# ymingxie/PARQ

Hardware: AMD Instinct MI355X
Metric: decoder-iterations/sec (10 views, 256 queries, d=256) (higher is better)
Workload: dtype f32 (cross-attention scores: fp16 hi.hi + MX-fp8 e4m3 cross terms; P V: fp16 probabilities and values with a self-consistent normaliser; fp32 accumulation — 4e-6..1.5e-5 from float64 at the outputs on the reference's fixtures, the reference's own fp32 run: 6e-5..1.4e-4; guarded: rows on too few keys

## Files before the change

__graft_entry__.py:

```python
from __future__ import annotations

import glob
import os
import subprocess
import sys

ROOT = os.path.dirname(os.path.abspath(__file__))
CSRC = os.path.join(ROOT, "parq_amd", "csrc")
OUT = os.path.join(ROOT, "parq_amd", "_C", "libparq_hip.so")
OUT_DEV = os.path.join(ROOT, "parq_amd", "_C", "libparq_hip_dev.so")


def _hipcc():
    for c in (os.environ.get("HIPCC"), "/opt/rocm/bin/hipcc", "hipcc"):
        if c and (os.path.isabs(c) and os.path.exists(c) or not os.path.isabs(c)):
            return c
    return "hipcc"


def _compile(out: str, objdir: str, flags, force: bool) -> None:
    srcs = sorted(glob.glob(os.path.join(CSRC, "*.hip")))
    deps = srcs + glob.glob(os.path.join(CSRC, "*.hpp")) + [os.path.join(ROOT, "include", "parq_hip.h")]
    os.makedirs(objdir, exist_ok=True)
    if not force and os.path.exists(out) and all(os.path.getmtime(out) >= os.path.getmtime(d) for d in deps):
        print("[build] up to date:", out)
        return
    objs = []
    procs = []
    for s in srcs:
        o = os.path.join(objdir, os.path.basename(s)[:-4] + ".o")
        objs.append(o)
        cmd = [_hipcc(), "--offload-arch=gfx950", "-O3", "-std=c++17", "-fPIC"] + list(flags) + ["-c", s, "-o", o]
        print("[build]", " ".join(cmd))
        procs.append((cmd, subprocess.Popen(cmd)))
    for cmd, p in procs:
        if p.wait() != 0:
            raise RuntimeError("hipcc failed: %s" % " ".join(cmd))
    cmd = [_hipcc(), "--offload-arch=gfx950", "-shared", "-fPIC", "-o", out] + objs
    print("[build]", " ".join(cmd))
    subprocess.check_call(cmd)


def build_dev(force: bool = False) -> None:
    extra = os.environ.get("PARQ_DEV_EXTRA_FLAGS", "").split()
    _compile(OUT_DEV, os.path.join(os.path.dirname(OUT_DEV), "dev"), ["-DPARQ_DEV_PROBES"] + extra, force or bool(extra))


def build(force: bool = False) -> None:
    _compile(OUT, os.path.dirname(OUT), [], force)
    if ROOT not in sys.path:
        sys.path.insert(0, ROOT)
    import parq_amd
    from parq_amd import _lib
    lib = _lib.load()
    print("[build] loaded", lib.parq_version().decode(), "with", len(_lib.SYMBOLS), "entry points")


def smoke() -> None:
    if ROOT not in sys.path:
        sys.path.insert(0, ROOT)
    import numpy as np
    import torch
    from parq_amd import synth
    from parq_amd.decoder import PARQDecoder
    from oracle import parq_oracle as O

    assert torch.cuda.is_available(), "smoke() needs a GPU"
    cfg = synth.decoder_cfg(dim=256, queries=64, heads=4, ffn=768, layers=2)
    W = synth.make_decoder_weights(cfg, seed=5)
    sc = synth.make_scene(55, B=1, V=2, h=60, w=80, C=256)
    dec = PARQDecoder(cfg).eval()
    sd = dec.state_dict()
    for k in sd:
        src = k.replace("parq_module.decoder.mlp_heads.", "mlp_heads.")
        sd[k] = torch.from_numpy(W[src]).reshape(sd[k].shape)
    dec.load_state_dict(sd, strict=True)
    dec = dec.cuda()
    t = lambda a: torch.from_numpy(a).cuda()
    with torch.no_grad():
        outs = dec(t(sc["tokens"]), t(sc["camera"]), t(sc["T_camera_pseudoCam"]), t(sc["T_world_pseudoCam"]),
                   t(sc["T_world_local"]))
    torch.cuda.synchronize()
    od = O.OracleDecoder(cfg, W, synth.SCANNET_MEAN_SIZES)
    forced = [O.normalize(o["coord_pos"].cpu(), cfg.TRANSFORMER.SCALE) for o in outs]
    with torch.no_grad():
        ref = od.forward(sc["tokens"], sc["camera"], sc["T_camera_pseudoCam"], sc["T_world_pseudoCam"],
                         sc["T_world_local"], forced_refs=forced)
    worst = 0.0
    for k, (a, b) in enumerate(zip(outs, ref)):
        for key in b:
            bb = b[key].numpy().astype(np.float64)
            err = np.abs(a[key].cpu().numpy().astype(np.float64) - bb) / np.maximum(1.0, np.abs(bb))
            worst = max(worst, float(err.max()))
    print("[smoke] max err vs oracle (teacher-forced, 2 iterations): %.3e" % worst)
    assert worst < 1e-4, worst


if __name__ == "__main__":
    build()
    if len(sys.argv) > 1 and sys.argv[1] == "dev":
        build_dev()
    if len(sys.argv) > 1 and sys.argv[1] == "smoke":
        smoke()
```

include/parq_hip.h:

```cpp
#ifndef PARQ_HIP_H
#define PARQ_HIP_H

#include <stddef.h>
#include <stdint.h>

#ifdef __cplusplus
extern "C" {
#endif

typedef struct parq_ctx *parq_handle;
typedef void *parq_stream;

enum {
    PARQ_OK = 0,
    PARQ_ERR_ARG = 1,
    PARQ_ERR_HIP = 2,
    PARQ_ERR_STATE = 3,
    PARQ_ERR_WORKSPACE = 4
};

typedef struct parq_config {
    int32_t dim;
    int32_t num_queries;
    int32_t num_classes;
    int32_t num_heads;
    int32_t ffn_dim;
    int32_t num_layers;
    int32_t share_weights;
    int32_t num_mean_sizes;
    float scale[6];
} parq_config;

typedef struct parq_scene {
    int32_t B, V, h, w;
    const float *tokens;
    const float *camera;
    const float *T_camera_pseudoCam;
    const float *T_world_pseudoCam;
    const float *T_world_local;
} parq_scene;

typedef struct parq_outputs {
    float *pred_logits;
    float *center_unnormalized;
    float *size_unnormalized;
    float *ortho6d;
    float *sem_cls_prob;
    float *coord_pos;
} parq_outputs;

const char *parq_last_error(void);
const char *parq_version(void);

int parq_create(const parq_config *cfg, parq_handle *out);
int parq_destroy(parq_handle h);

int parq_set_weight(parq_handle h, const char *name, const float *dev, int64_t numel);
size_t parq_packed_weights_bytes(parq_handle h);
int parq_pack_weights(parq_handle h, void *arena, size_t arena_bytes, parq_stream stream);

int parq_set_attention_mode(parq_handle h, int32_t mode);

enum { PARQ_TOKENS_F32 = 0, PARQ_TOKENS_F16 = 1, PARQ_TOKENS_BF16 = 2 };
int parq_set_token_type(parq_handle h, int32_t type);
int parq_set_head_tiers(parq_handle h, uint32_t safe_mask, int32_t poison_on_peaked);
int parq_set_seam_fusion(parq_handle h, int32_t on);
int parq_set_range_mirror(parq_handle h, int32_t *host_visible_flag);
int32_t parq_mirror_take(int32_t *host_visible_flag);
int parq_set_progress(parq_handle h, int32_t *host_visible_word, int32_t epoch);

size_t parq_workspace_bytes(parq_handle h, int32_t B, int32_t V, int32_t hh, int32_t ww);

int parq_forward(parq_handle h, const parq_scene *scene, void *workspace, size_t workspace_bytes,
                 const parq_outputs *outs, parq_stream stream);

typedef struct parq_graph *parq_graph_t;
int parq_forward_capture(parq_handle h, int32_t B, int32_t V, int32_t hh, int32_t ww, void *workspace, size_t workspace_bytes,
                         parq_stream stream, parq_graph_t *out);
int parq_forward_replay(parq_handle h, parq_graph_t g, const parq_scene *scene, void *workspace, size_t workspace_bytes,
                        const parq_outputs *outs, parq_stream stream);
int64_t parq_graph_nodes(parq_graph_t g);
int parq_graph_destroy(parq_graph_t g);

int parq_prepare(parq_handle h, const parq_scene *scene, void *workspace, size_t workspace_bytes,
                 parq_stream stream);
int parq_iterate(parq_handle h, const parq_scene *scene, void *workspace, size_t workspace_bytes,
                 int32_t layer_num, const float *ref_in, const parq_outputs *outs, float *ref_out,
                 parq_stream stream);

size_t parq_shard_exchange_floats(parq_handle h, int32_t B, int32_t which);
int parq_iterate_sharded(parq_handle h, const parq_scene *scene, void *workspace, size_t workspace_bytes, int32_t layer_num,
                         int32_t phase, const float *ref_in, const parq_outputs *outs, float *ref_out, const float *xchg_in,
                         float *xchg_out, int32_t nranks, parq_stream stream);

int parq_workspace_lookup(parq_handle h, int32_t B, int32_t V, int32_t hh, int32_t ww, const char *name,
                          size_t *offset_floats, size_t *numel);

enum {
    PARQ_PROF_KV_PROJ = 0, PARQ_PROF_PROJECT_SAMPLE = 1, PARQ_PROF_CROSS_ATTN = 2,
    PARQ_PROF_SELF_ATTN = 3, PARQ_PROF_LINEAR = 4, PARQ_PROF_OTHER = 5, PARQ_PROF_MERGE = 6, PARQ_PROF_COUNT = 7
};
int parq_profile_enable(parq_handle h, int32_t on);
int parq_profile_read(parq_handle h, int32_t which, double *total_ms, int64_t *launches);

typedef struct parq_output_grads {
    const float *pred_logits, *center_unnormalized, *size_unnormalized, *ortho6d;
} parq_output_grads;
int parq_set_dropout(parq_handle h, float p, uint32_t seed);
int parq_set_backward_batched(parq_handle h, int32_t on);
int parq_k_dropout_mask(parq_handle h, int32_t iteration, int32_t site, int64_t rows, int64_t cols, float *out,
                        parq_stream stream);
size_t parq_train_workspace_bytes(parq_handle h, int32_t B, int32_t V, int32_t hh, int32_t ww);
size_t parq_grad_arena_bytes(parq_handle h);
int parq_forward_train(parq_handle h, const parq_scene *scene, void *workspace, size_t workspace_bytes,
                       const parq_outputs *outs, parq_stream stream);
int parq_wait_iteration(parq_handle h, int32_t k);
int parq_backward(parq_handle h, const parq_scene *scene, void *workspace, size_t workspace_bytes, const parq_outputs *outs,
                  const parq_output_grads *grads, float *grad_arena, float *d_tokens, parq_stream stream);
int parq_arena_lookup(parq_handle h, const char *name, int64_t *offset, int64_t *rows, int64_t *cols, int64_t *ld);
int parq_grad_bucket(parq_handle h, int32_t bucket, int64_t *offset, int64_t *count);
int parq_backward_wait_bucket(parq_handle h, int32_t bucket, parq_stream stream);
int parq_set_backward_streams(parq_handle h, int32_t n);
int parq_set_deterministic(parq_handle h, int32_t on);

enum { PARQ_RAYPE_NCHW_OUT = 1, PARQ_RAYPE_NO_HIDDEN = 2, PARQ_RAYPE_WEIGHTS_CACHED = 4, PARQ_RAYPE_OUT_F16 = 8, PARQ_RAYPE_OUT_BF16 = 16 };
size_t parq_ray_pe_workspace_bytes(int32_t B, int32_t V, int32_t hh, int32_t ww, int32_t C, int32_t num_samples);
size_t parq_ray_pe_workspace_bytes_flags(int32_t B, int32_t V, int32_t hh, int32_t ww, int32_t C, int32_t num_samples,
                                         int32_t flags);
int parq_ray_pe(const float *camera, const float *T_camera_pseudoCam, const float *T_world_pseudoCam,
                const float *T_world_local, const float *w1, const float *b1, const float *w2, const float *b2,
                const float *scale6_host, float min_depth, float max_depth, int32_t num_samples, int32_t B,
                int32_t V, int32_t hh, int32_t ww, int32_t C, const float *features_nchw, float *tokens_out,
                int32_t flags, void *workspace, size_t workspace_bytes, parq_stream stream);

typedef struct {
    const float *level[4];
    int32_t h[4], w[4];
    int32_t layer;
} parq_fpn_levels;
int parq_ray_pe_fpn(const float *camera, const float *T_camera_pseudoCam, const float *T_world_pseudoCam,
                    const float *T_world_local, const float *w1, const float *b1, const float *w2, const float *b2,
                    const float *scale6_host, float min_depth, float max_depth, int32_t num_samples, int32_t B,
                    int32_t V, int32_t hh, int32_t ww, int32_t C, const parq_fpn_levels *levels, float *tokens_out,
                    int32_t flags, void *workspace, size_t workspace_bytes, parq_stream stream);
int parq_fpn_backward(const float *d_tokens, int32_t B, int32_t V, int32_t C, const parq_fpn_levels *levels, float *const d_level[4],
                      parq_stream stream);

size_t parq_ray_pe_backward_workspace_bytes(int32_t B, int32_t V, int32_t hh, int32_t ww, int32_t C, int32_t num_samples);
int parq_ray_pe_backward(const float *camera, const float *T_camera_pseudoCam, const float *T_world_pseudoCam,
                         const float *T_world_local, const float *w2, const float *scale6_host, float min_depth,
                         float max_depth, int32_t num_samples, int32_t B, int32_t V, int32_t hh, int32_t ww, int32_t C,
                         const float *d_tokens, const void *fwd_workspace, void *bwd_workspace, size_t bwd_workspace_bytes,
                         float *dw1, float *db1, float *dw2, float *db2, float *d_features_nchw, parq_stream stream);
enum { PARQ_RAYPE_BWD_DETERMINISTIC = 1 };
size_t parq_ray_pe_backward_workspace_bytes_flags(int32_t B, int32_t V, int32_t hh, int32_t ww, int32_t C, int32_t num_samples,
                                                  int32_t flags);
int parq_ray_pe_backward_flags(const float *camera, const float *T_camera_pseudoCam, const float *T_world_pseudoCam,
                               const float *T_world_local, const float *w2, const float *scale6_host, float min_depth,
                               float max_depth, int32_t num_samples, int32_t B, int32_t V, int32_t hh, int32_t ww, int32_t C,
                               const float *d_tokens, const void *fwd_workspace, void *bwd_workspace, size_t bwd_workspace_bytes,
                               float *dw1, float *db1, float *dw2, float *db2, float *d_features_nchw, int32_t flags,
                               parq_stream stream);

int parq_parse_pred(const float *center, const float *size, const float *ortho6d, const float *sem_cls_prob, int32_t B,
                    int32_t Q, int32_t num_classes, const float *track_scale6_host, int32_t for_vis, int32_t enable_nms,
                    float *obbs_out, unsigned char *mask_out, parq_stream stream);

int parq_obb_iou(const double *boxes_a, int64_t n_a_total, const double *boxes_b, int64_t n_b_total, const int64_t *segments,
                 int32_t S, int64_t total_pairs, double *iou3d_out, double *iou2d_out, parq_stream stream);

int parq_set_loss(const float *pred_logits, const float *center_unnormalized, const float *size_unnormalized, const float *ortho6d,
                  int32_t I, int32_t B, int32_t Q, int32_t num_classes, const float *t_center, const float *t_size, const float *t_rot,
                  const int32_t *t_label, const int32_t *t_sym, int32_t nmax, const int32_t *pairs, const float *pair_coef, int32_t P,
                  const float *row_weight, const float *class_weight, const float *loss_weight4_host, float *terms, float *g_logits,
                  float *g_center, float *g_size, float *g_ortho6d, int32_t *class_scratch, parq_stream stream);
enum { PARQ_SETLOSS_DETERMINISTIC = 1 };
size_t parq_set_loss_scratch_bytes(int32_t I, int32_t B, int32_t Q, int32_t P, int32_t flags);
int parq_set_loss_flags(const float *pred_logits, const float *center_unnormalized, const float *size_unnormalized, const float *ortho6d,
                        int32_t I, int32_t B, int32_t Q, int32_t num_classes, const float *t_center, const float *t_size, const float *t_rot,
                        const int32_t *t_label, const int32_t *t_sym, int32_t nmax, const int32_t *pairs, const float *pair_coef, int32_t P,
                        const float *row_weight, const float *class_weight, const float *loss_weight4_host, float *terms, float *g_logits,
                        float *g_center, float *g_size, float *g_ortho6d, int32_t *class_scratch, int32_t flags, parq_stream stream);


int parq_k_project_sample(const float *tokens, const float *T_camera_local, const float *camera,
                          const float *ref, const float *scale6_host, int32_t B, int32_t V, int32_t hh,
                          int32_t ww, int32_t C, int32_t Q, float *tgt, float *coord_pos,
                          parq_stream stream);

int parq_k_camera_local(const float *T_cp, const float *T_wp, const float *T_wl, int32_t B, int32_t V,
                        float *T_cl, parq_stream stream);

int parq_k_linear(const float *X, const float *X2, const float *W, const float *bias, const float *R,
                  float *Y, int32_t M, int32_t N, int32_t K, int32_t relu, parq_stream stream);

int parq_k_linear_half(const float *X, const float *X2, const float *W, const float *bias, const float *R,
                       float *Y, int32_t M, int32_t N, int32_t K, int32_t relu, void *scratch, size_t scratch_bytes,
                       parq_stream stream);

size_t parq_k_attention_scratch_bytes(int32_t B, int32_t H, int32_t Lq, int32_t Lk, int32_t dh);
int parq_k_attention(const float *q, const float *k, const float *v, float *out, int32_t B, int32_t H,
                     int32_t Lq, int32_t Lk, int32_t dh, void *scratch, size_t scratch_bytes,
                     parq_stream stream);

size_t parq_k_attention_split_scratch_bytes(int32_t B, int32_t H, int32_t Lq, int32_t Lk);
int parq_k_attention_split(const float *q, const float *k, const float *v, float *out, int32_t B, int32_t H,
                           int32_t Lq, int32_t Lk, void *scratch, size_t scratch_bytes, parq_stream stream);

int parq_k_attention_split8(const float *q, const float *k, const float *v, float *out, int32_t B, int32_t H,
                            int32_t Lq, int32_t Lk, void *scratch, size_t scratch_bytes, parq_stream stream);

size_t parq_k_attention_split256_scratch_bytes(int32_t B, int32_t H, int32_t Lq, int32_t Lk);
int parq_k_attention_split256(const float *q, const float *k, const float *v, float *out, int32_t B, int32_t H,
                              int32_t Lq, int32_t Lk, void *scratch, size_t scratch_bytes, parq_stream stream);

size_t parq_k_attention_half_scratch_bytes(int32_t B, int32_t H, int32_t Lq, int32_t Lk);
int parq_k_attention_half(const float *q, const float *k, const float *v, float *out, int32_t B, int32_t H,
                          int32_t Lq, int32_t Lk, int32_t bf16, void *scratch, size_t scratch_bytes,
                          parq_stream stream);

int parq_k_layernorm(const float *X, const float *gamma, const float *beta, float *Y, int32_t M,
                     int32_t C, float eps, parq_stream stream);

#ifdef __cplusplus
}
#endif
#endif
```

parq_amd/_lib.py:

```python
from __future__ import annotations

import ctypes as C
import os

import torch

_HERE = os.path.dirname(os.path.abspath(__file__))
LIB_PATH = os.path.join(_HERE, "_C", "libparq_hip.so")
DEV_LIB_PATH = os.path.join(_HERE, "_C", "libparq_hip_dev.so")

PROF_KV_PROJ, PROF_PROJECT_SAMPLE, PROF_CROSS_ATTN, PROF_SELF_ATTN, PROF_LINEAR, PROF_OTHER, PROF_MERGE = range(7)
PROF_NAMES = ["kv_proj", "project_sample", "cross_attn", "self_attn", "linear", "other", "cross_attn_merge"]


class ParqConfig(C.Structure):
    _fields_ = [("dim", C.c_int32), ("num_queries", C.c_int32), ("num_classes", C.c_int32),
                ("num_heads", C.c_int32), ("ffn_dim", C.c_int32), ("num_layers", C.c_int32),
                ("share_weights", C.c_int32), ("num_mean_sizes", C.c_int32), ("scale", C.c_float * 6)]


class ParqScene(C.Structure):
    _fields_ = [("B", C.c_int32), ("V", C.c_int32), ("h", C.c_int32), ("w", C.c_int32),
                ("tokens", C.c_void_p), ("camera", C.c_void_p), ("T_camera_pseudoCam", C.c_void_p),
                ("T_world_pseudoCam", C.c_void_p), ("T_world_local", C.c_void_p)]


class ParqOutputs(C.Structure):
    _fields_ = [("pred_logits", C.c_void_p), ("center_unnormalized", C.c_void_p),
                ("size_unnormalized", C.c_void_p), ("ortho6d", C.c_void_p),
                ("sem_cls_prob", C.c_void_p), ("coord_pos", C.c_void_p)]


class ParqOutputGrads(C.Structure):
    _fields_ = [("pred_logits", C.c_void_p), ("center_unnormalized", C.c_void_p),
                ("size_unnormalized", C.c_void_p), ("ortho6d", C.c_void_p)]


class ParqFpnLevels(C.Structure):
    _fields_ = [("level", C.c_void_p * 4), ("h", C.c_int32 * 4), ("w", C.c_int32 * 4), ("layer", C.c_int32)]


_vp, _i32, _i64, _sz, _f = C.c_void_p, C.c_int32, C.c_int64, C.c_size_t, C.c_float
SYMBOLS = {
    "parq_last_error": (C.c_char_p, []),
    "parq_version": (C.c_char_p, []),
    "parq_create": (C.c_int, [C.POINTER(ParqConfig), C.POINTER(_vp)]),
    "parq_destroy": (C.c_int, [_vp]),
    "parq_set_weight": (C.c_int, [_vp, C.c_char_p, _vp, _i64]),
    "parq_packed_weights_bytes": (_sz, [_vp]),
    "parq_pack_weights": (C.c_int, [_vp, _vp, _sz, _vp]),
    "parq_workspace_bytes": (_sz, [_vp, _i32, _i32, _i32, _i32]),
    "parq_forward": (C.c_int, [_vp, C.POINTER(ParqScene), _vp, _sz, C.POINTER(ParqOutputs), _vp]),
    "parq_forward_capture": (C.c_int, [_vp, _i32, _i32, _i32, _i32, _vp, _sz, _vp, C.POINTER(_vp)]),
    "parq_forward_replay": (C.c_int, [_vp, _vp, C.POINTER(ParqScene), _vp, _sz, C.POINTER(ParqOutputs), _vp]),
    "parq_graph_nodes": (_i64, [_vp]),
    "parq_graph_destroy": (C.c_int, [_vp]),
    "parq_prepare": (C.c_int, [_vp, C.POINTER(ParqScene), _vp, _sz, _vp]),
    "parq_iterate": (C.c_int, [_vp, C.POINTER(ParqScene), _vp, _sz, _i32, _vp, C.POINTER(ParqOutputs), _vp, _vp]),
    "parq_workspace_lookup": (C.c_int, [_vp, _i32, _i32, _i32, _i32, C.c_char_p, C.POINTER(_sz), C.POINTER(_sz)]),
    "parq_set_attention_mode": (C.c_int, [_vp, _i32]),
    "parq_set_token_type": (C.c_int, [_vp, _i32]),
    "parq_set_head_tiers": (C.c_int, [_vp, C.c_uint32, _i32]),
    "parq_set_seam_fusion": (C.c_int, [_vp, _i32]),
    "parq_set_range_mirror": (C.c_int, [_vp, _vp]),
    "parq_mirror_take": (_i32, [_vp]),
    "parq_set_progress": (C.c_int, [_vp, _vp, _i32]),
    "parq_shard_exchange_floats": (_sz, [_vp, _i32, _i32]),
    "parq_iterate_sharded": (C.c_int, [_vp, C.POINTER(ParqScene), _vp, _sz, _i32, _i32, _vp, C.POINTER(ParqOutputs), _vp, _vp, _vp, _i32, _vp]),
    "parq_profile_enable": (C.c_int, [_vp, _i32]),
    "parq_profile_read": (C.c_int, [_vp, _i32, C.POINTER(C.c_double), C.POINTER(_i64)]),
    "parq_set_dropout": (C.c_int, [_vp, _f, C.c_uint32]),
    "parq_set_backward_batched": (C.c_int, [_vp, _i32]),
    "parq_k_dropout_mask": (C.c_int, [_vp, _i32, _i32, _i64, _i64, _vp, _vp]),
    "parq_train_workspace_bytes": (_sz, [_vp, _i32, _i32, _i32, _i32]),
    "parq_grad_arena_bytes": (_sz, [_vp]),
    "parq_forward_train": (C.c_int, [_vp, C.POINTER(ParqScene), _vp, _sz, C.POINTER(ParqOutputs), _vp]),
    "parq_wait_iteration": (C.c_int, [_vp, C.c_int32]),
    "parq_backward": (C.c_int, [_vp, C.POINTER(ParqScene), _vp, _sz, C.POINTER(ParqOutputs), C.POINTER(ParqOutputGrads), _vp, _vp, _vp]),
    "parq_arena_lookup": (C.c_int, [_vp, C.c_char_p, C.POINTER(_i64), C.POINTER(_i64), C.POINTER(_i64), C.POINTER(_i64)]),
    "parq_grad_bucket": (C.c_int, [_vp, _i32, C.POINTER(_i64), C.POINTER(_i64)]),
    "parq_backward_wait_bucket": (C.c_int, [_vp, _i32, _vp]),
    "parq_set_backward_streams": (C.c_int, [_vp, _i32]),
    "parq_set_deterministic": (C.c_int, [_vp, _i32]),
    "parq_ray_pe_workspace_bytes": (_sz, [_i32, _i32, _i32, _i32, _i32, _i32]),
    "parq_ray_pe_workspace_bytes_flags": (_sz, [_i32, _i32, _i32, _i32, _i32, _i32, _i32]),
    "parq_ray_pe": (C.c_int, [_vp, _vp, _vp, _vp, _vp, _vp, _vp, _vp, C.POINTER(_f), _f, _f, _i32, _i32, _i32, _i32, _i32, _i32,
                              _vp, _vp, _i32, _vp, _sz, _vp]),
    "parq_ray_pe_fpn": (C.c_int, [_vp, _vp, _vp, _vp, _vp, _vp, _vp, _vp, C.POINTER(_f), _f, _f, _i32, _i32, _i32, _i32, _i32, _i32,
                                  C.POINTER(ParqFpnLevels), _vp, _i32, _vp, _sz, _vp]),
    "parq_fpn_backward": (C.c_int, [_vp, _i32, _i32, _i32, C.POINTER(ParqFpnLevels), C.POINTER(_vp), _vp]),
    "parq_ray_pe_backward_workspace_bytes": (_sz, [_i32, _i32, _i32, _i32, _i32, _i32]),
    "parq_ray_pe_backward": (C.c_int, [_vp, _vp, _vp, _vp, _vp, C.POINTER(_f), _f, _f, _i32, _i32, _i32, _i32, _i32, _i32, _vp, _vp, _vp,
                                       _sz, _vp, _vp, _vp, _vp, _vp, _vp]),
    "parq_ray_pe_backward_workspace_bytes_flags": (_sz, [_i32, _i32, _i32, _i32, _i32, _i32, _i32]),
    "parq_ray_pe_backward_flags": (C.c_int, [_vp, _vp, _vp, _vp, _vp, C.POINTER(_f), _f, _f, _i32, _i32, _i32, _i32, _i32, _i32, _vp, _vp,
                                             _vp, _sz, _vp, _vp, _vp, _vp, _vp, _i32, _vp]),
    "parq_parse_pred": (C.c_int, [_vp, _vp, _vp, _vp, _i32, _i32, _i32, C.POINTER(_f), _i32, _i32, _vp, _vp, _vp]),
    "parq_obb_iou": (C.c_int, [_vp, _i64, _vp, _i64, _vp, _i32, _i64, _vp, _vp, _vp]),
    "parq_set_loss": (C.c_int, [_vp, _vp, _vp, _vp, _i32, _i32, _i32, _i32, _vp, _vp, _vp, _vp, _vp, _i32, _vp, _vp, _i32, _vp, _vp,
                                C.POINTER(_f), _vp, _vp, _vp, _vp, _vp, _vp, _vp]),
    "parq_set_loss_scratch_bytes": (_sz, [_i32, _i32, _i32, _i32, _i32]),
    "parq_set_loss_flags": (C.c_int, [_vp, _vp, _vp, _vp, _i32, _i32, _i32, _i32, _vp, _vp, _vp, _vp, _vp, _i32, _vp, _vp, _i32, _vp, _vp,
                                      C.POINTER(_f), _vp, _vp, _vp, _vp, _vp, _vp, _i32, _vp]),
    "parq_k_project_sample": (C.c_int, [_vp, _vp, _vp, _vp, C.POINTER(_f), _i32, _i32, _i32, _i32, _i32, _i32, _vp, _vp, _vp]),
    "parq_k_camera_local": (C.c_int, [_vp, _vp, _vp, _i32, _i32, _vp, _vp]),
    "parq_k_linear": (C.c_int, [_vp, _vp, _vp, _vp, _vp, _vp, _i32, _i32, _i32, _i32, _vp]),
    "parq_k_linear_half": (C.c_int, [_vp, _vp, _vp, _vp, _vp, _vp, _i32, _i32, _i32, _i32, _vp, _sz, _vp]),
    "parq_k_attention_scratch_bytes": (_sz, [_i32, _i32, _i32, _i32, _i32]),
    "parq_k_attention": (C.c_int, [_vp, _vp, _vp, _vp, _i32, _i32, _i32, _i32, _i32, _vp, _sz, _vp]),
    "parq_k_attention_split_scratch_bytes": (_sz, [_i32, _i32, _i32, _i32]),
    "parq_k_attention_split": (C.c_int, [_vp, _vp, _vp, _vp, _i32, _i32, _i32, _i32, _vp, _sz, _vp]),
    "parq_k_attention_split8": (C.c_int, [_vp, _vp, _vp, _vp, _i32, _i32, _i32, _i32, _vp, _sz, _vp]),
    "parq_k_attention_split256_scratch_bytes": (_sz, [_i32, _i32, _i32, _i32]),
    "parq_k_attention_split256": (C.c_int, [_vp, _vp, _vp, _vp, _i32, _i32, _i32, _i32, _vp, _sz, _vp]),
    "parq_k_attention_half_scratch_bytes": (_sz, [_i32, _i32, _i32, _i32]),
    "parq_k_attention_half": (C.c_int, [_vp, _vp, _vp, _vp, _i32, _i32, _i32, _i32, _i32, _vp, _sz, _vp]),
    "parq_k_layernorm": (C.c_int, [_vp, _vp, _vp, _vp, _i32, _i32, _f, _vp]),
}

_lib = None


def use_dev_library():
    global LIB_PATH
    if _lib is not None:
        raise RuntimeError("parq_amd: use_dev_library() must be called before the library is first loaded")
    LIB_PATH = DEV_LIB_PATH


def is_dev_library():
    return LIB_PATH == DEV_LIB_PATH


def load():
    global _lib
    if _lib is not None:
        return _lib
    if not os.path.exists(LIB_PATH):
        raise RuntimeError(
            "parq_amd: HIP extension %s is missing. Build it with "
            "`python -c 'import __graft_entry__ as g; g.build()'` (needs hipcc, --offload-arch=gfx950). "
            "There is no CPU fallback." % LIB_PATH)
    lib = C.CDLL(LIB_PATH)
    for name, (res, args) in SYMBOLS.items():
        try:
            fn = getattr(lib, name)
        except AttributeError as e:
            raise RuntimeError("parq_amd: %s does not export %s (stale build?)" % (LIB_PATH, name)) from e
        fn.restype = res
        fn.argtypes = args
    _lib = lib
    return lib


def check(rc: int, what: str):
    if rc != 0:
        msg = load().parq_last_error().decode("utf-8", "replace")
        raise RuntimeError("parq_amd: %s failed (code %d): %s" % (what, rc, msg))


def ptr(t):
    if t is None:
        return None
    assert t.is_cuda and t.dtype == torch.float32 and t.is_contiguous(), \
        "expected a contiguous float32 CUDA tensor, got %s %s contiguous=%s" % (t.device, t.dtype, t.is_contiguous())
    return C.c_void_p(t.data_ptr())


def token_ptr(t):
    assert t.is_cuda and t.dtype in (torch.float32, torch.float16, torch.bfloat16) and t.is_contiguous(), \
        "expected contiguous float32 / float16 / bfloat16 CUDA tokens, got %s %s contiguous=%s" % (t.device, t.dtype, t.is_contiguous())
    return C.c_void_p(t.data_ptr())


def stream_ptr():
    return C.c_void_p(torch.cuda.current_stream().cuda_stream)
```

parq_amd/csrc/api.hip:

```cpp
#include "../../include/parq_hip.h"
#include "common.hpp"

#include <cmath>
#include <cstdarg>
#include <cstdio>
#include <cstring>
#include <map>
#include <string>
#include <vector>

using namespace parq;

namespace {
constexpr float kPeakyL = 256.f;

thread_local char g_err[512] = "";

int fail(int code, const char* fmt, ...) {
    va_list ap;
    va_start(ap, fmt);
    vsnprintf(g_err, sizeof(g_err), fmt, ap);
    va_end(ap);
    return code;
}
// ... 1523 lines not shown
    if (!h->iter_recorded[k]) return fail(PARQ_ERR_STATE, "parq_wait_iteration: no parq_forward_train has been enqueued");
    HIPCHK(hipEventSynchronize(h->iter_done[k]));
    return PARQ_OK;
}

int parq_backward(parq_handle h, const parq_scene* scene, void* workspace, size_t workspace_bytes, const parq_outputs* outs,
                  const parq_output_grads* g, float* grad_arena, float* d_tokens, parq_stream stream) {
    if (!h || !workspace || !outs || !g || !grad_arena) return fail(PARQ_ERR_ARG, "NULL argument");
    if (h->tok_type != kTokF32) return fail(PARQ_ERR_ARG, "parq_backward reads fp32 tokens only: set token type 0");
    if (!h->packed) return fail(PARQ_ERR_STATE, "parq_pack_weights must be called first");
    int rc = check_scene(h, scene);
    if (rc) return rc;
    Workspace ws;
    carve_workspace(h, scene->B, scene->V, scene->h, scene->w, &ws);
    if (workspace_bytes < (size_t)ws.train_total * sizeof(float)) return fail(PARQ_ERR_WORKSPACE, "training workspace too small");
    float* wsp = (float*)workspace;
    hipStream_t s = (hipStream_t)stream;
    const int64_t M = (int64_t)scene->B * h->Q;
    const int64_t N = (int64_t)scene->V * scene->h * scene->w;
    if (h->deterministic && h->dh == 32) return fail(PARQ_ERR_ARG, "deterministic mode: no fixed-order attention backward at head dim 32");
    DetScope det(h->deterministic ? wsp + ws.g_det : nullptr, ws.g_det_floats);
    HIPCHK(hipMemsetAsync(grad_arena, 0, (size_t)h->ar.rowmajor_total * sizeof(float), s));
    if (!ws.bwd_batched) HIPCHK(hipMemsetAsync(wsp + ws.g_kv, 0, (size_t)h->nl * scene->B * 2 * N * h->C * sizeof(float), s));
    if (d_tokens) HIPCHK(hipMemsetAsync(d_tokens, 0, (size_t)scene->B * N * h->C * sizeof(float), s));
    auto iter_io = [&](int k) {
        BwdIO io;
        io.g_logits = g->pred_logits ? g->pred_logits + k * M * h->ncls : nullptr;
        io.g_center = g->center_unnormalized ? g->center_unnormalized + k * M * 3 : nullptr;
        io.g_size = g->size_unnormalized ? g->size_unnormalized + k * M * 3 : nullptr;
        io.g_rot = g->ortho6d ? g->ortho6d + k * M * 6 : nullptr;
        io.center = outs->center_unnormalized + k * M * 3;
        io.size = outs->size_unnormalized + k * M * 3;
        return io;
    };
    for (int i = 0; i < 2; ++i)
        if (!h->bucket_done[i]) HIPCHK(hipEventCreateWithFlags(&h->bucket_done[i], hipEventDisableTiming));
    auto finish = [&](bool early_too) -> int {
        const int r = do_backward_kvproj(h, scene, wsp, ws, grad_arena, d_tokens, s);
        if (r) return r;
        if (early_too) HIPCHK(hipEventRecord(h->bucket_done[0], s));
        HIPCHK(hipEventRecord(h->bucket_done[1], s));
        h->bucket_recorded = true;
        return PARQ_OK;
    };
    if (!ws.bwd_batched) {
        for (int k = h->I - 1; k >= 0; --k) {
            rc = do_backward_iter(h, scene, wsp, ws, k, iter_io(k), grad_arena, d_tokens, s);
            if (rc) return rc;
        }
        return finish(true);
    }
    const int I = h->I, B = scene->B, C = h->C, H = h->H, dh = h->dh, Q = h->Q;
    rc = do_backward_transposes(h, wsp, ws, 0, s);
    if (rc) return rc;
    const int ns = h->profiling ? 1 : ws.g_sets;
    if (ns > 1 && !h->fork_ev) {
        HIPCHK(hipEventCreateWithFlags(&h->fork_ev, hipEventDisableTiming));
        for (int i = 0; i < 7; ++i) {
            HIPCHK(hipStreamCreateWithFlags(&h->aux_stream[i], hipStreamNonBlocking));
            HIPCHK(hipEventCreateWithFlags(&h->join_ev[i], hipEventDisableTiming));
        }
    }
    auto run_phase = [&](int phase) -> int {
        if (ns > 1) {
            HIPCHK(hipEventRecord(h->fork_ev, s));
            for (int i = 0; i + 1 < ns; ++i) HIPCHK(hipStreamWaitEvent(h->aux_stream[i], h->fork_ev, 0));
        }
        int r = PARQ_OK;
        for (int k = I - 1, n = 0; k >= 0 && r == PARQ_OK; --k, ++n) {
            const int set = n % ns;
            r = do_backward_iter(h, scene, wsp, ws, k, iter_io(k), grad_arena, d_tokens, set == 0 ? s : h->aux_stream[set - 1], phase, set);
        }
        for (int i = 0; i + 1 < ns; ++i) {
            const hipError_t e1 = hipEventRecord(h->join_ev[i], h->aux_stream[i]);
            const hipError_t e2 = hipStreamWaitEvent(s, h->join_ev[i], 0);
            if (r == PARQ_OK && (e1 != hipSuccess || e2 != hipSuccess)) r = fail(PARQ_ERR_HIP, "joining the backward's auxiliary streams failed");
        }
        return r;
    };
    rc = run_phase(1);
    if (rc) return rc;
    HIPCHK(hipEventRecord(h->bucket_done[0], s));
    {
        int64_t q_off[16], lse_off[16];
        uint32_t seeds[16];
        for (int k = 0; k < I; ++k) {
            q_off[k] = ws.shift(k);
            lse_off[k] = ws.shift(k);
            seeds[k] = h->site_seed(k, 2);
        }
        const float* kv = wsp + (h->cache_mode() ? ws.kv_train : ws.kv);
        float* gkv = wsp + ws.g_kv;
        const int64_t MC = M * C;
        HIPCHK(hipMemsetAsync(wsp + ws.g_dq, 0, (size_t)I * MC * sizeof(float), s));
        HIPCHK(launch_attn_bwd_batched(wsp + ws.qc, q_off, (int64_t)Q * C, dh, C, kv, 2 * N * C, N * dh, dh, kv + (int64_t)H * N * dh,
                                       2 * N * C, N * dh, dh, wsp + ws.g_do, MC, (int64_t)Q * C, dh, C, wsp + ws.lse_c, lse_off,
                                       wsp + ws.g_Dall, (int64_t)B * H * flash_lq_pad(Q), wsp + ws.g_dq, MC, (int64_t)Q * C, dh, C, gkv,
                                       2 * N * C, dh, 2 * C, gkv + C, 2 * N * C, dh, 2 * C, B, H, Q, (int)N, dh, I, s, wsp + ws.g_dqp,
                                       h->drop_p, seeds, reinterpret_cast<unsigned int*>(wsp + ws.g_bs),
                                       reinterpret_cast<unsigned int*>(wsp + ws.g_kvmax), wsp + ws.g_pack, wsp + ws.g_mat,
                                       bwd_reads_cache(h, ws) ? reinterpret_cast<const void*>(wsp + ws.kvc) : nullptr,
                                       h->terms_for(N, true, bwd_reads_cache(h, ws)), h->kind()));
        if (dh == 256) {
            HIPCHK(hipMemsetAsync(wsp + ws.g_kvmax, 0, sizeof(unsigned int), s));
            HIPCHK(launch_absmax(gkv, (int64_t)B * 2 * N * C, reinterpret_cast<unsigned int*>(wsp + ws.g_kvmax), s));
        }
    }
    rc = run_phase(2);
    if (rc) return rc;
    return finish(false);
}

int parq_grad_bucket(parq_handle h, int32_t bucket, int64_t* offset, int64_t* count) {
    if (!h || !offset || !count || bucket < 0 || bucket > 1) return fail(PARQ_ERR_ARG, "bad argument");
    const Arena& ar = h->ar;
    const bool two = h->nl == 1 && ar.early_end > ar.early_begin;
    if (bucket == 0) { *offset = two ? ar.early_begin : 0; *count = two ? ar.early_end - ar.early_begin : 0; }
    else { *offset = 0; *count = two ? ar.early_begin : ar.rowmajor_total; }
    return PARQ_OK;
}

int parq_backward_wait_bucket(parq_handle h, int32_t bucket, parq_stream stream) {
    if (!h || bucket < 0 || bucket > 1) return fail(PARQ_ERR_ARG, "bad argument");
    if (!h->bucket_recorded) return fail(PARQ_ERR_STATE, "parq_backward_wait_bucket: no parq_backward has been enqueued");
    HIPCHK(hipStreamWaitEvent((hipStream_t)stream, h->bucket_done[bucket], 0));
    return PARQ_OK;
}

int parq_arena_lookup(parq_handle h, const char* name, int64_t* offset, int64_t* rows, int64_t* cols, int64_t* ld) {
    if (!h || !name || !offset || !rows || !cols || !ld) return fail(PARQ_ERR_ARG, "NULL argument");
    const int64_t C = h->C, F = h->F, Q = h->Q, ncls = h->ncls;
    const Arena& ar = h->ar;
    struct E { std::string n; int64_t off, r, c; };
    std::vector<E> t;
    for (int li = 0; li < h->nl; ++li) {
        const LayerW& L = ar.layers[li];
        const std::string p = "parq_module.decoder.layers." + std::to_string(li) + ".";
        t.push_back({p + "self_attn.in_proj_weight", L.self_in_w, 3 * C, C}); t.push_back({p + "self_attn.in_proj_bias", L.self_in_b, 1, 3 * C});
        t.push_back({p + "self_attn.out_proj.weight", L.self_out_w, C, C}); t.push_back({p + "self_attn.out_proj.bias", L.self_out_b, 1, C});
        t.push_back({p + "multihead_attn.in_proj_weight", L.cross_in_w, 3 * C, C}); t.push_back({p + "multihead_attn.in_proj_bias", L.cross_in_b, 1, 3 * C});
        t.push_back({p + "multihead_attn.out_proj.weight", L.cross_out_w, C, C}); t.push_back({p + "multihead_attn.out_proj.bias", L.cross_out_b, 1, C});
        t.push_back({p + "linear1.weight", L.lin1_w, F, C}); t.push_back({p + "linear1.bias", L.lin1_b, 1, F});
        t.push_back({p + "linear2.weight", L.lin2_w, C, F}); t.push_back({p + "linear2.bias", L.lin2_b, 1, C});
        t.push_back({p + "norm1.weight", L.n1_w, 1, C}); t.push_back({p + "norm1.bias", L.n1_b, 1, C});
        t.push_back({p + "norm2.weight", L.n2_w, 1, C}); t.push_back({p + "norm2.bias", L.n2_b, 1, C});
        t.push_back({p + "norm3.weight", L.n3_w, 1, C}); t.push_back({p + "norm3.bias", L.n3_b, 1, C});
    }
    const std::string d = "parq_module.decoder.";
    const std::string hc = "mlp_heads.center_head.layers.", hr = "mlp_heads.rotation_head.layers.";
    t.push_back({"refpoint.weight", ar.refpoint, Q, 3});
    t.push_back({d + "position_encoder.0.weight", ar.pe0_w, C, 384}); t.push_back({d + "position_encoder.0.bias", ar.pe0_b, 1, C});
    t.push_back({d + "position_encoder.2.weight", ar.pe2_w, C, C}); t.push_back({d + "position_encoder.2.bias", ar.pe2_b, 1, C});
    t.push_back({hc + "0.weight", ar.heads1_w, C, C}); t.push_back({hr + "0.weight", ar.heads1_w + C * C, C, C});
    t.push_back({"mlp_heads.sem_cls_head.layers.0.weight", ar.heads1_w + 2 * C * C, ncls, C});
    t.push_back({"mlp_heads.size_head.layers.0.weight", ar.heads1_w + (2 * C + ncls) * C, 3, C});
    t.push_back({"mlp_heads.sem_cls_head.layers.0.bias", ar.heads1_b + 2 * C, 1, ncls});
    t.push_back({"mlp_heads.size_head.layers.0.bias", ar.heads1_b + 2 * C + ncls, 1, 3});
    t.push_back({hc + "1.weight", ar.gn1_g, 1, C}); t.push_back({hr + "1.weight", ar.gn1_g + C, 1, C});
    t.push_back({hc + "1.bias", ar.gn1_b, 1, C}); t.push_back({hr + "1.bias", ar.gn1_b + C, 1, C});
    t.push_back({hc + "4.weight", ar.heads2_w, C, C}); t.push_back({hr + "4.weight", ar.heads2_w + C * C, C, C});
    t.push_back({hc + "5.weight", ar.gn2_g, 1, C}); t.push_back({hr + "5.weight", ar.gn2_g + C, 1, C});
    t.push_back({hc + "5.bias", ar.gn2_b, 1, C}); t.push_back({hr + "5.bias", ar.gn2_b + C, 1, C});
    t.push_back({hc + "8.weight", ar.heads3_w, 3, C}); t.push_back({hr + "8.weight", ar.heads3_w + 6 * C, 6, C});
    t.push_back({hc + "8.bias", ar.heads3_b, 1, 3}); t.push_back({hr + "8.bias", ar.heads3_b + 6, 1, 6});
    for (const E& e : t)
        if (e.n == name) { *offset = e.off; *rows = e.r; *cols = e.c; *ld = e.c; return PARQ_OK; }
    return fail(PARQ_ERR_ARG, "unknown tensor '%s'", name);
}

int parq_profile_enable(parq_handle h, int32_t on) {
    if (!h) return fail(PARQ_ERR_ARG, "NULL handle");
    h->profiling = on != 0;
    return PARQ_OK;
}

int parq_profile_read(parq_handle h, int32_t which, double* total_ms, int64_t* launches) {
    if (!h || which < 0 || which >= PARQ_PROF_COUNT) return fail(PARQ_ERR_ARG, "bad argument");
    for (auto& e : h->events) {
        HIPCHK(hipEventSynchronize(e.b));
        float ms = 0.f;
        HIPCHK(hipEventElapsedTime(&ms, e.a, e.b));
        h->prof_ms[e.which] += ms;
        h->prof_n[e.which] += 1;
        (void)hipEventDestroy(e.a);
        (void)hipEventDestroy(e.b);
    }
    h->events.clear();
    if (total_ms) *total_ms = h->prof_ms[which];
    if (launches) *launches = h->prof_n[which];
    h->prof_ms[which] = 0;
    h->prof_n[which] = 0;
    return PARQ_OK;
}


int parq_k_camera_local(const float* T_cp, const float* T_wp, const float* T_wl, int32_t B, int32_t V, float* T_cl,
                        parq_stream stream) {
    if (!T_cp || !T_wp || !T_wl || !T_cl || B < 1 || V < 1) return fail(PARQ_ERR_ARG, "bad argument");
    HIPCHK(launch_camera_local(T_cp, T_wp, T_wl, B, V, T_cl, (hipStream_t)stream));
    return PARQ_OK;
}

int parq_k_project_sample(const float* tokens, const float* T_cl, const float* camera, const float* ref,
                          const float* scale6_host, int32_t B, int32_t V, int32_t hh, int32_t ww, int32_t C, int32_t Q,
                          float* tgt, float* coord_pos, parq_stream stream) {
    if (!tokens || !T_cl || !camera || !ref || !scale6_host || !tgt) return fail(PARQ_ERR_ARG, "NULL argument");
    if (B < 1 || V < 1 || hh < 2 || ww < 2 || Q < 1 || C % 4 != 0 || C > 1024) return fail(PARQ_ERR_ARG, "bad dims");
    ScaleBox sb;
    for (int i = 0; i < 3; ++i) { sb.lo[i] = scale6_host[2 * i]; sb.hi[i] = scale6_host[2 * i + 1]; }
    HIPCHK(launch_project_sample(tokens, T_cl, camera, ref, sb, B, V, hh, ww, C, Q, tgt, coord_pos, (hipStream_t)stream));
    return PARQ_OK;
}

int parq_k_linear(const float* X, const float* X2, const float* W, const float* bias, const float* R, float* Y,
                  int32_t M, int32_t N, int32_t K, int32_t relu, parq_stream stream) {
    if (!X || !W || !Y || M < 1 || N < 1 || K < 32 || K % 32 != 0) return fail(PARQ_ERR_ARG, "bad argument (K must be a multiple of 32)");
    LinearArgs a = lin(X, K, W, K, bias, Y, N, M, N, K);
    a.X2 = X2; a.ldx2 = K; a.x2_ncols = N;
    a.R = R; a.ldr = N; a.relu = relu;
    HIPCHK(launch_linear(a, 1, (hipStream_t)stream));
    return PARQ_OK;
}

int parq_k_linear_half(const float* X, const float* X2, const float* W, const float* bias, const float* R, float* Y,
                       int32_t M, int32_t N, int32_t K, int32_t relu, void* scratch, size_t scratch_bytes, parq_stream stream) {
    if (!X || !W || !Y || !scratch || M < 16 || N < 16 || M % 16 != 0 || N % 16 != 0 || !(K == 1024 || K == 768))
        return fail(PARQ_ERR_ARG, "bad argument (K in {1024, 768}, M and N multiples of 16)");
    if (scratch_bytes < ((size_t)N * K + N) * sizeof(float) || (reinterpret_cast<uintptr_t>(scratch) & 15u))
        return fail(PARQ_ERR_ARG, "scratch: N * K * 4 + N * 4 bytes, 16-byte aligned");
    float* wh = static_cast<float*>(scratch);
    float* sc = wh + (size_t)N * K;
    HIPCHK(launch_pack_w_half(W, K, N, K, wh, sc, (hipStream_t)stream));
    LinearArgs a = lin(X, K, W, K, bias, Y, N, M, N, K);
    a.X2 = X2; a.ldx2 = K; a.x2_ncols = N;
    a.R = R; a.ldr = N; a.relu = relu;
    a.Wh = wh; a.wh_scale = sc;
    const hipError_t e = launch_chain_linear(a, 1, (hipStream_t)stream);
    if (e == hipErrorNotSupported) return fail(PARQ_ERR_ARG, "no fp16 x 3 tile for this combination of addend / bias / ReLU / residual");
    HIPCHK(e);
    return PARQ_OK;
}

size_t parq_k_attention_scratch_bytes(int32_t B, int32_t H, int32_t Lq, int32_t Lk, int32_t dh) {
    const int ns = flash_pick_splits(B, H, Lq, Lk, dh, device_num_cus());
    return flash_scratch_bytes(B, H, Lq, dh, ns);
}

int parq_k_attention(const float* q, const float* k, const float* v, float* out, int32_t B, int32_t H, int32_t Lq,
                     int32_t Lk, int32_t dh, void* scratch, size_t scratch_bytes, parq_stream stream) {
    if (!q || !k || !v || !out || !scratch) return fail(PARQ_ERR_ARG, "NULL argument");
    if (!(dh == 32 || dh == 64 || dh == 128 || dh == 256) || B < 1 || H < 1 || Lq < 1 || Lk < 1) return fail(PARQ_ERR_ARG, "bad dims");
    FlashArgs fa;
    memset(&fa, 0, sizeof(fa));
    const int64_t C = (int64_t)H * dh;
    fa.B = B; fa.H = H; fa.Lq = Lq; fa.Lk = Lk; fa.dh = dh;
    fa.q = q; fa.q_batch = Lq * C; fa.q_head = dh; fa.q_row = C;
    fa.k = k; fa.k_batch = Lk * C; fa.k_head = dh; fa.k_row = C;
    fa.v = v; fa.v_batch = Lk * C; fa.v_head = dh; fa.v_row = C;
    fa.out = out; fa.out_batch = Lq * C; fa.out_row = C;
    fa.nsplit = flash_pick_splits(B, H, Lq, Lk, dh, device_num_cus());
    if (scratch_bytes < flash_scratch_bytes(B, H, Lq, dh, fa.nsplit)) return fail(PARQ_ERR_WORKSPACE, "attention scratch too small");
    const int64_t lp = flash_lq_pad(Lq);
    fa.o_part = (float*)scratch;
    fa.m_part = fa.o_part + (int64_t)B * H * fa.nsplit * dh * lp;
    fa.l_part = fa.m_part + (int64_t)B * H * fa.nsplit * lp;
    HIPCHK(launch_flash(fa, (hipStream_t)stream));
    HIPCHK(launch_flash_merge(fa, (hipStream_t)stream));
    return PARQ_OK;
}

size_t parq_k_attention_split_scratch_bytes(int32_t B, int32_t H, int32_t Lq, int32_t Lk) {
    const int ns = flash_split_pick_splits(B, H, Lq, Lk, device_num_cus());
    return flash_scratch_bytes(B, H, Lq, 64, ns) + kvsplit_cache_bytes(B, H, Lk) + 256;
}

int parq_k_attention_split(const float* q, const float* k, const float* v, float* out, int32_t B, int32_t H, int32_t Lq,
                           int32_t Lk, void* scratch, size_t scratch_bytes, parq_stream stream) {
    if (!q || !k || !v || !out || !scratch) return fail(PARQ_ERR_ARG, "NULL argument");
    if (B < 1 || H < 1 || Lq < 1 || Lk < 1) return fail(PARQ_ERR_ARG, "bad dims");
    if (scratch_bytes < parq_k_attention_split_scratch_bytes(B, H, Lq, Lk)) return fail(PARQ_ERR_WORKSPACE, "attention scratch too small");
    hipStream_t s = (hipStream_t)stream;
    const int dh = 64;
    const int64_t C = (int64_t)H * dh;
    FlashArgs fa;
    memset(&fa, 0, sizeof(fa));
    fa.B = B; fa.H = H; fa.Lq = Lq; fa.Lk = Lk; fa.dh = dh;
    fa.q = q; fa.q_batch = Lq * C; fa.q_head = dh; fa.q_row = C;
    fa.out = out; fa.out_batch = Lq * C; fa.out_row = C;
    fa.nsplit = flash_split_pick_splits(B, H, Lq, Lk, device_num_cus());
    const int64_t lp = flash_lq_pad(Lq);
    char* base = (char*)scratch;
    int* flag = (int*)base;
    char* cache = base + 256;
    fa.o_part = (float*)(cache + kvsplit_cache_bytes(B, H, Lk));
    fa.m_part = fa.o_part + (int64_t)B * H * fa.nsplit * dh * lp;
    fa.l_part = fa.m_part + (int64_t)B * H * fa.nsplit * lp;
    HIPCHK(hipMemsetAsync(flag, 0, 256, s));
    HIPCHK(launch_kvsplit_convert(k, v, Lk * C, dh, C, Lk * C, dh, C, B, H, Lk, cache, flag, s));
    HIPCHK(launch_flash_split(fa, cache, s));
    HIPCHK(launch_flash_merge(fa, s));
    return PARQ_OK;
}

int parq_k_attention_split8(const float* q, const float* k, const float* v, float* out, int32_t B, int32_t H, int32_t Lq,
                            int32_t Lk, void* scratch, size_t scratch_bytes, parq_stream stream) {
    if (!q || !k || !v || !out || !scratch) return fail(PARQ_ERR_ARG, "NULL argument");
    if (B < 1 || H < 1 || Lq < 1 || Lk < 1) return fail(PARQ_ERR_ARG, "bad dims");
    if (!flash_split8_supported(64, Lk)) return fail(PARQ_ERR_ARG, "attention mode 4 needs a key count that is a multiple of 64");
    if (scratch_bytes < parq_k_attention_split_scratch_bytes(B, H, Lq, Lk)) return fail(PARQ_ERR_WORKSPACE, "attention scratch too small");
    hipStream_t s = (hipStream_t)stream;
    const int dh = 64;
    const int64_t C = (int64_t)H * dh;
    FlashArgs fa;
    memset(&fa, 0, sizeof(fa));
    fa.B = B; fa.H = H; fa.Lq = Lq; fa.Lk = Lk; fa.dh = dh;
    fa.q = q; fa.q_batch = Lq * C; fa.q_head = dh; fa.q_row = C;
    fa.out = out; fa.out_batch = Lq * C; fa.out_row = C;
    fa.nsplit = flash_split_pick_splits(B, H, Lq, Lk, device_num_cus());
    const int64_t lp = flash_lq_pad(Lq);
    char* cache = (char*)scratch + 256;
    fa.o_part = (float*)(cache + kvsplit_cache_bytes(B, H, Lk));
    fa.m_part = fa.o_part + (int64_t)B * H * fa.nsplit * dh * lp;
    fa.l_part = fa.m_part + (int64_t)B * H * fa.nsplit * lp;
    HIPCHK(launch_kvsplit8_convert(k, v, Lk * C, dh, C, Lk * C, dh, C, B, H, Lk, cache, s));
    HIPCHK(launch_flash_split8(fa, cache, s));
    HIPCHK(launch_flash_merge(fa, s));
    return PARQ_OK;
}

size_t parq_k_attention_split256_scratch_bytes(int32_t B, int32_t H, int32_t Lq, int32_t Lk) {
    const int ns = flash_split256_pick_splits(B, H, Lq, Lk, device_num_cus());
    return flash_scratch_bytes(B, H, Lq, 256, ns) + kvsplit_cache_bytes(B, 4 * H, Lk) + 256;
}

int parq_k_attention_split256(const float* q, const float* k, const float* v, float* out, int32_t B, int32_t H, int32_t Lq,
                              int32_t Lk, void* scratch, size_t scratch_bytes, parq_stream stream) {
    if (!q || !k || !v || !out || !scratch) return fail(PARQ_ERR_ARG, "NULL argument");
    if (B < 1 || H < 1 || Lq < 1 || Lk < 1) return fail(PARQ_ERR_ARG, "bad dims");
    if (scratch_bytes < parq_k_attention_split256_scratch_bytes(B, H, Lq, Lk)) return fail(PARQ_ERR_WORKSPACE, "attention scratch too small");
    hipStream_t s = (hipStream_t)stream;
    const int dh = 256;
    const int64_t C = (int64_t)H * dh;
    FlashArgs fa;
    memset(&fa, 0, sizeof(fa));
    fa.B = B; fa.H = H; fa.Lq = Lq; fa.Lk = Lk; fa.dh = dh;
    fa.q = q; fa.q_batch = Lq * C; fa.q_head = dh; fa.q_row = C;
    fa.out = out; fa.out_batch = Lq * C; fa.out_row = C;
    fa.nsplit = flash_split256_pick_splits(B, H, Lq, Lk, device_num_cus());
    const int64_t lp = flash_lq_pad(Lq);
    char* base = (char*)scratch;
    int* flag = (int*)base;
    char* cache = base + 256;
    fa.o_part = (float*)(cache + kvsplit_cache_bytes(B, 4 * H, Lk));
    fa.m_part = fa.o_part + (int64_t)B * H * fa.nsplit * dh * lp;
    fa.l_part = fa.m_part + (int64_t)B * H * fa.nsplit * lp;
    HIPCHK(hipMemsetAsync(flag, 0, 256, s));
    HIPCHK(launch_kvsplit_convert(k, v, Lk * C, 64, C, Lk * C, 64, C, B, 4 * H, Lk, cache, flag, s));
    HIPCHK(launch_flash_split256(fa, cache, s));
    HIPCHK(launch_flash_merge(fa, s));
    return PARQ_OK;
}

size_t parq_k_attention_half_scratch_bytes(int32_t B, int32_t H, int32_t Lq, int32_t Lk) {
    return parq_k_attention_split_scratch_bytes(B, H, Lq, Lk);
}

int parq_k_attention_half(const float* q, const float* k, const float* v, float* out, int32_t B, int32_t H, int32_t Lq,
                          int32_t Lk, int32_t bf16, void* scratch, size_t scratch_bytes, parq_stream stream) {
    if (!q || !k || !v || !out || !scratch) return fail(PARQ_ERR_ARG, "NULL argument");
    if (B < 1 || H < 1 || Lq < 1 || Lk < 1) return fail(PARQ_ERR_ARG, "bad dims");
    if (scratch_bytes < parq_k_attention_half_scratch_bytes(B, H, Lq, Lk)) return fail(PARQ_ERR_WORKSPACE, "attention scratch too small");
    hipStream_t s = (hipStream_t)stream;
    const int dh = 64, kind = bf16 ? kBF16 : kF16;
    const int64_t C = (int64_t)H * dh;
    FlashArgs fa;
    memset(&fa, 0, sizeof(fa));
    fa.B = B; fa.H = H; fa.Lq = Lq; fa.Lk = Lk; fa.dh = dh;
    fa.q = q; fa.q_batch = Lq * C; fa.q_head = dh; fa.q_row = C;
    fa.out = out; fa.out_batch = Lq * C; fa.out_row = C;
    fa.nsplit = flash_split_pick_splits(B, H, Lq, Lk, device_num_cus());
    const int64_t lp = flash_lq_pad(Lq);
    char* base = (char*)scratch;
    int* flag = (int*)base;
    char* cache = base + 256;
    fa.o_part = (float*)(cache + kvsplit_cache_bytes(B, H, Lk, 3));
    fa.m_part = fa.o_part + (int64_t)B * H * fa.nsplit * dh * lp;
    fa.l_part = fa.m_part + (int64_t)B * H * fa.nsplit * lp;
    HIPCHK(hipMemsetAsync(flag, 0, 256, s));
    HIPCHK(launch_kvsplit_convert(k, v, Lk * C, dh, C, Lk * C, dh, C, B, H, Lk, cache, flag, s, 1, kind));
    HIPCHK(launch_flash_split(fa, cache, s, 1, kind));
    HIPCHK(launch_flash_merge(fa, s));
    return PARQ_OK;
}

static int64_t raype_align(int64_t x) { return (x + 63) / 64 * 64; }

static bool raype_keeps_hidden(int32_t C, int32_t num_samples, int32_t flags) {
    return !((flags & PARQ_RAYPE_NO_HIDDEN) && C == 256 && num_samples == 64);
}
size_t parq_ray_pe_workspace_bytes_flags(int32_t B, int32_t V, int32_t hh, int32_t ww, int32_t C, int32_t num_samples, int32_t flags) {
    if (B < 1 || V < 1 || hh < 1 || ww < 1 || C < 1 || num_samples < 1) return 0;
    const int64_t M = (int64_t)B * V * hh * ww, K1 = 3 * (int64_t)num_samples;
    const bool fused = (C == 256 && num_samples == 64);
    const int64_t floats = (raype_keeps_hidden(C, num_samples, flags) ? raype_align(M * C) : 0) + raype_align(C * K1) +
                           2 * raype_align((int64_t)C * C) + raype_align(2 * ((int64_t)B * V * 12 + num_samples)) +
                           (fused ? 0 : raype_align(M * K1));
    return (size_t)floats * sizeof(float);
}
size_t parq_ray_pe_workspace_bytes(int32_t B, int32_t V, int32_t hh, int32_t ww, int32_t C, int32_t num_samples) {
    return parq_ray_pe_workspace_bytes_flags(B, V, hh, ww, C, num_samples, 0);
}

static int ray_pe_impl(const float* camera, const float* T_cp, const float* T_wp, const float* T_wl, const float* w1,
                       const float* b1, const float* w2, const float* b2, const float* scale6_host, float min_depth,
                       float max_depth, int32_t num_samples, int32_t B, int32_t V, int32_t hh, int32_t ww, int32_t C,
                       const float* features_nchw, const FpnDev* fpn, float* tokens_out, int32_t flags, void* workspace,
                       size_t workspace_bytes, parq_stream stream) {
    const int32_t nchw_out = flags & PARQ_RAYPE_NCHW_OUT;
    const int out16 = (flags & PARQ_RAYPE_OUT_F16) ? kTokF16 : (flags & PARQ_RAYPE_OUT_BF16) ? kTokBF16 : kTokF32;
    if ((flags & PARQ_RAYPE_OUT_F16) && (flags & PARQ_RAYPE_OUT_BF16)) return fail(PARQ_ERR_ARG, "ray-PE: one 16-bit output type at a time");
    if (out16 != kTokF32 && (nchw_out || !(flags & PARQ_RAYPE_NO_HIDDEN)))
        return fail(PARQ_ERR_ARG, "ray-PE: 16-bit tokens are an inference output (no-hidden flag, channels-last)");
    if (!camera || !T_cp || !T_wp || !T_wl || !w1 || !b1 || !w2 || !b2 || !scale6_host || !tokens_out || !workspace)
        return fail(PARQ_ERR_ARG, "NULL argument");
    if (B < 1 || V < 1 || hh < 1 || ww < 1 || num_samples < 1) return fail(PARQ_ERR_ARG, "bad dims");
    if ((3 * num_samples) % 64 != 0 || C % 64 != 0) return fail(PARQ_ERR_ARG, "3*num_samples and C must be multiples of 64");
    if (!(max_depth > min_depth && min_depth > 0.f)) return fail(PARQ_ERR_ARG, "need 0 < min_depth < max_depth");
    if (workspace_bytes < parq_ray_pe_workspace_bytes_flags(B, V, hh, ww, C, num_samples, flags)) return fail(PARQ_ERR_WORKSPACE, "ray-PE workspace too small");
    const int64_t M64 = (int64_t)B * V * hh * ww;
    if (M64 > INT32_MAX) return fail(PARQ_ERR_ARG, "too many tokens");
    const int M = (int)M64, K1 = 3 * num_samples;
    hipStream_t s = (hipStream_t)stream;
    float* wsp = (float*)workspace;
    const bool keep = raype_keeps_hidden(C, num_samples, flags);
    float* Hd = keep ? wsp : nullptr;
    float* W1s = wsp + (keep ? raype_align((int64_t)M * C) : 0);
    float* W2s = W1s + raype_align((int64_t)C * K1);
    float* W2f = W2s + raype_align((int64_t)C * C);
    double* tabs = reinterpret_cast<double*>(W2f + raype_align((int64_t)C * C));
    float* P = reinterpret_cast<float*>(tabs) + raype_align(2 * ((int64_t)B * V * 12 + num_samples));
    char* w1hi = (char*)W1s; char* w1lo = w1hi + (size_t)C * K1 * 2;
    char* w2hi = (char*)W2s; char* w2lo = w2hi + (size_t)C * C * 2;
    const bool cached = (flags & PARQ_RAYPE_WEIGHTS_CACHED) != 0;
    if (!cached) {
        HIPCHK(launch_split_f32(w1, w1hi, w1lo, (int64_t)C * K1, s));
        HIPCHK(launch_split_f32(w2, w2hi, w2lo, (int64_t)C * C, s));
    }
    if (C == 256 && num_samples == 64) {
        static const int two = [] { const char* e = dev_env("PARQ_RAYPE_TWO_KERNELS"); return e && e[0] == '1' ? 1 : 0; }();
        if (two && !Hd) return fail(PARQ_ERR_ARG, "the two-kernel form needs the hidden region (do not pass the no-hidden flag)");
        if (two && fpn) return fail(PARQ_ERR_ARG, "the two-kernel development form of the ray-PE does not take pyramids");
        HIPCHK(launch_raype_fused(camera, T_cp, T_wp, T_wl, scale6_host, min_depth, max_depth, B, V, hh, ww, w1hi, w1lo, b1,
                                  w2hi, w2lo, b2, features_nchw, Hd, tabs, tabs + (int64_t)B * V * 12, tokens_out,
                                  nchw_out ? 1 : 0, s, W2f, two | (cached ? 2 : 0), out16, fpn));
        return PARQ_OK;
    }
    if (nchw_out) return fail(PARQ_ERR_ARG, "NCHW output needs the fused path (C = 256, 64 samples)");
    HIPCHK(launch_raype_points(camera, T_cp, T_wp, T_wl, scale6_host, min_depth, max_depth, B, V, hh, ww, num_samples, P, s));
    HIPCHK(launch_gemm_split(P, K1, w1hi, w1lo, b1, Hd, C, M, C, K1, 1, nullptr, 1, s));
    HIPCHK(launch_gemm_split(Hd, C, w2hi, w2lo, b2, tokens_out, C, M, C, C, 0, features_nchw, hh * ww, s, nullptr, 1.f, nullptr, 0, out16,
                             fpn));
    return PARQ_OK;
}

int parq_ray_pe(const float* camera, const float* T_cp, const float* T_wp, const float* T_wl, const float* w1,
                const float* b1, const float* w2, const float* b2, const float* scale6_host, float min_depth,
                float max_depth, int32_t num_samples, int32_t B, int32_t V, int32_t hh, int32_t ww, int32_t C,
                const float* features_nchw, float* tokens_out, int32_t flags, void* workspace, size_t workspace_bytes,
                parq_stream stream) {
    return ray_pe_impl(camera, T_cp, T_wp, T_wl, w1, b1, w2, b2, scale6_host, min_depth, max_depth, num_samples, B, V, hh, ww, C,
                       features_nchw, nullptr, tokens_out, flags, workspace, workspace_bytes, stream);
}

static int fpn_check(const parq_fpn_levels* lv, int32_t hh, int32_t ww, int32_t C, FpnDev& f) {
    if (!lv) return fail(PARQ_ERR_ARG, "NULL pyramid");
    if (C < 4 || C % 4 != 0 || (C / 4) % 16 != 0)
        return fail(PARQ_ERR_ARG, "pyramid: C = %d must be 4 levels of a multiple of 16 channels", (int)C);
    if (lv->layer < 0 || lv->layer > 3) return fail(PARQ_ERR_ARG, "pyramid: layer %d outside 0..3", (int)lv->layer);
    for (int l = 0; l < 4; ++l) {
        if (!lv->level[l]) return fail(PARQ_ERR_ARG, "pyramid: level %d is NULL", l);
        if (lv->h[l] < 1 || lv->w[l] < 1) return fail(PARQ_ERR_ARG, "pyramid: level %d is %d x %d", l, (int)lv->h[l], (int)lv->w[l]);
        if ((int64_t)lv->h[l] * lv->w[l] * (C / 4) > INT32_MAX / 4) return fail(PARQ_ERR_ARG, "pyramid: level %d too large", l);
        f.lv[l] = lv->level[l];
        f.h[l] = lv->h[l];
        f.w[l] = lv->w[l];
    }
    if (lv->h[lv->layer] != hh || lv->w[lv->layer] != ww)
        return fail(PARQ_ERR_ARG, "pyramid: target level %d is %d x %d but the tokens are %d x %d per view", (int)lv->layer,
                    (int)lv->h[lv->layer], (int)lv->w[lv->layer], (int)hh, (int)ww);
    f.layer = lv->layer;
    f.cl = C / 4;
    return PARQ_OK;
}

int parq_ray_pe_fpn(const float* camera, const float* T_cp, const float* T_wp, const float* T_wl, const float* w1,
                    const float* b1, const float* w2, const float* b2, const float* scale6_host, float min_depth,
                    float max_depth, int32_t num_samples, int32_t B, int32_t V, int32_t hh, int32_t ww, int32_t C,
                    const parq_fpn_levels* levels, float* tokens_out, int32_t flags, void* workspace, size_t workspace_bytes,
                    parq_stream stream) {
    if (flags & PARQ_RAYPE_NCHW_OUT) return fail(PARQ_ERR_ARG, "pyramid: channels-last tokens only (no NCHW output)");
    FpnDev f;
    if (int rc = fpn_check(levels, hh, ww, C, f); rc != PARQ_OK) return rc;
    return ray_pe_impl(camera, T_cp, T_wp, T_wl, w1, b1, w2, b2, scale6_host, min_depth, max_depth, num_samples, B, V, hh, ww, C,
                       nullptr, &f, tokens_out, flags, workspace, workspace_bytes, stream);
}

int parq_fpn_backward(const float* d_tokens, int32_t B, int32_t V, int32_t C, const parq_fpn_levels* levels, float* const d_level[4],
                      parq_stream stream) {
    if (!d_tokens || !d_level || !d_level[0] || !d_level[1] || !d_level[2] || !d_level[3]) return fail(PARQ_ERR_ARG, "NULL argument");
    if (B < 1 || V < 1) return fail(PARQ_ERR_ARG, "bad dims");
    if (!levels) return fail(PARQ_ERR_ARG, "NULL pyramid");
    const int l = levels->layer;
    if (l < 0 || l > 3) return fail(PARQ_ERR_ARG, "pyramid: layer %d outside 0..3", l);
    FpnDev f;
    if (int rc = fpn_check(levels, levels->h[l], levels->w[l], C, f); rc != PARQ_OK) return rc;
    if ((int64_t)B * V * levels->h[l] * levels->w[l] * C > INT32_MAX) return fail(PARQ_ERR_ARG, "too many tokens");
    HIPCHK(launch_fpn_backward(d_tokens, B * V, f, d_level, (hipStream_t)stream));
    return PARQ_OK;
}

size_t parq_ray_pe_backward_workspace_bytes_flags(int32_t B, int32_t V, int32_t hh, int32_t ww, int32_t C, int32_t num_samples,
                                                  int32_t flags) {
    if (B < 1 || V < 1 || hh < 1 || ww < 1 || C < 1 || num_samples < 1 || (flags & ~PARQ_RAYPE_BWD_DETERMINISTIC)) return 0;
    const int64_t M = (int64_t)B * V * hh * ww, K1 = 3 * (int64_t)num_samples;
    const int64_t det = (flags & PARQ_RAYPE_BWD_DETERMINISTIC) ? raype_align(det_scratch_floats(0, 0)) : 0;
    return (size_t)(raype_align(M * K1) + raype_align(M * C) + raype_align((int64_t)C * C) + det) * sizeof(float);
}
size_t parq_ray_pe_backward_workspace_bytes(int32_t B, int32_t V, int32_t hh, int32_t ww, int32_t C, int32_t num_samples) {
    return parq_ray_pe_backward_workspace_bytes_flags(B, V, hh, ww, C, num_samples, 0);
}

int parq_ray_pe_backward(const float* camera, const float* T_cp, const float* T_wp, const float* T_wl, const float* w2,
                         const float* scale6_host, float min_depth, float max_depth, int32_t num_samples, int32_t B, int32_t V,
                         int32_t hh, int32_t ww, int32_t C, const float* d_tokens, const void* fwd_workspace, void* bwd_workspace,
                         size_t bwd_workspace_bytes, float* dw1, float* db1, float* dw2, float* db2, float* d_features_nchw,
                         parq_stream stream) {
    return parq_ray_pe_backward_flags(camera, T_cp, T_wp, T_wl, w2, scale6_host, min_depth, max_depth, num_samples, B, V, hh, ww, C,
                                      d_tokens, fwd_workspace, bwd_workspace, bwd_workspace_bytes, dw1, db1, dw2, db2, d_features_nchw, 0,
                                      stream);
}

int parq_ray_pe_backward_flags(const float* camera, const float* T_cp, const float* T_wp, const float* T_wl, const float* w2,
                               const float* scale6_host, float min_depth, float max_depth, int32_t num_samples, int32_t B, int32_t V,
                               int32_t hh, int32_t ww, int32_t C, const float* d_tokens, const void* fwd_workspace, void* bwd_workspace,
                               size_t bwd_workspace_bytes, float* dw1, float* db1, float* dw2, float* db2, float* d_features_nchw,
                               int32_t flags, parq_stream stream) {
    if (flags & ~PARQ_RAYPE_BWD_DETERMINISTIC) return fail(PARQ_ERR_ARG, "unknown ray-PE backward flags 0x%x", (unsigned)flags);
    if (!camera || !T_cp || !T_wp || !T_wl || !w2 || !scale6_host || !d_tokens || !fwd_workspace || !bwd_workspace || !dw1 || !db1 ||
        !dw2 || !db2)
        return fail(PARQ_ERR_ARG, "NULL argument");
    if (B < 1 || V < 1 || hh < 1 || ww < 1 || num_samples < 1 || (3 * num_samples) % 64 != 0 || C % 64 != 0) return fail(PARQ_ERR_ARG, "bad dims");
    if (bwd_workspace_bytes < parq_ray_pe_backward_workspace_bytes_flags(B, V, hh, ww, C, num_samples, flags))
        return fail(PARQ_ERR_WORKSPACE, "ray-PE backward workspace too small");
    const int64_t M64 = (int64_t)B * V * hh * ww;
    if (M64 > INT32_MAX) return fail(PARQ_ERR_ARG, "too many tokens");
    const int M = (int)M64, K1 = 3 * num_samples;
    hipStream_t s = (hipStream_t)stream;
    const float* Hd = (const float*)fwd_workspace;
    float* P = (float*)bwd_workspace;
    float* gHd = P + raype_align((int64_t)M * K1);
    float* W2T = gHd + raype_align((int64_t)M * C);
    const bool det_on = (flags & PARQ_RAYPE_BWD_DETERMINISTIC) != 0;
    DetScope det(det_on ? W2T + raype_align((int64_t)C * C) : nullptr, det_on ? det_scratch_floats(0, 0) : 0);
    HIPCHK(hipMemsetAsync(db2, 0, (size_t)C * sizeof(float), s));
    HIPCHK(hipMemsetAsync(db1, 0, (size_t)C * sizeof(float), s));
    HIPCHK(launch_colsum(d_tokens, C, M, C, db2, 1, s));
    HIPCHK(hipMemsetAsync(dw2, 0, (size_t)C * C * sizeof(float), s));
    HIPCHK(launch_gemm_tn(d_tokens, C, Hd, C, dw2, C, M, C, C, 1, s));
    HIPCHK(launch_transpose(w2, C, W2T, C, C, C, s));
    {
        LinearArgs a = lin(d_tokens, C, W2T, C, nullptr, gHd, C, M, C, C);
        a.relu_mask = Hd; a.ldmask = C;
        HIPCHK(launch_linear(a, 1, s));
    }
    HIPCHK(launch_colsum(gHd, C, M, C, db1, 1, s));
    HIPCHK(launch_raype_points(camera, T_cp, T_wp, T_wl, scale6_host, min_depth, max_depth, B, V, hh, ww, num_samples, P, s));
    HIPCHK(hipMemsetAsync(dw1, 0, (size_t)C * K1 * sizeof(float), s));
    HIPCHK(launch_gemm_tn(gHd, C, P, K1, dw1, K1, M, C, K1, 1, s));
    if (d_features_nchw) {
        const int hw = hh * ww;
        for (int i = 0; i < B * V; ++i)
            HIPCHK(launch_transpose(d_tokens + (int64_t)i * hw * C, C, d_features_nchw + (int64_t)i * C * hw, hw, hw, C, s));
    }
    return PARQ_OK;
}

int parq_parse_pred(const float* center, const float* size, const float* ortho6d, const float* sem_cls_prob, int32_t B, int32_t Q,
                    int32_t num_classes, const float* track_scale6_host, int32_t for_vis, int32_t enable_nms, float* obbs_out,
                    unsigned char* mask_out, parq_stream stream) {
    if (!center || !size || !ortho6d || !sem_cls_prob || !track_scale6_host || !obbs_out || !mask_out) return fail(PARQ_ERR_ARG, "NULL argument");
    if (B < 1 || Q < 1 || Q > 1024 || num_classes < 2) return fail(PARQ_ERR_ARG, "bad dims (1 <= Q <= 1024)");
    HIPCHK(launch_parse_pred(center, size, ortho6d, sem_cls_prob, B, Q, num_classes, num_classes - 1, track_scale6_host, for_vis,
                             enable_nms, obbs_out, mask_out, (hipStream_t)stream));
    return PARQ_OK;
}

int parq_obb_iou(const double* boxes_a, int64_t n_a_total, const double* boxes_b, int64_t n_b_total, const int64_t* segments, int32_t S,
                 int64_t total_pairs, double* iou3d_out, double* iou2d_out, parq_stream stream) {
    if (S < 0 || total_pairs < 0 || n_a_total < 0 || n_b_total < 0) return fail(PARQ_ERR_ARG, "parq_obb_iou: negative count");
    if (S == 0 || total_pairs == 0) return PARQ_OK;
    if (!boxes_a || !boxes_b || !segments || !iou3d_out) return fail(PARQ_ERR_ARG, "parq_obb_iou: NULL argument");
    if (n_a_total < 1 || n_b_total < 1) return fail(PARQ_ERR_ARG, "parq_obb_iou: %lld pairs of no boxes", (long long)total_pairs);
    if ((total_pairs + 63) / 64 > (int64_t)INT32_MAX) return fail(PARQ_ERR_ARG, "parq_obb_iou: too many pairs");
    HIPCHK(launch_obb_iou(boxes_a, boxes_b, segments, S, total_pairs, n_a_total, n_b_total, iou3d_out, iou2d_out, (hipStream_t)stream));
    return PARQ_OK;
}

int parq_set_loss(const float* pred_logits, const float* center_unnormalized, const float* size_unnormalized, const float* ortho6d,
                  int32_t I, int32_t B, int32_t Q, int32_t num_classes, const float* t_center, const float* t_size, const float* t_rot,
                  const int32_t* t_label, const int32_t* t_sym, int32_t nmax, const int32_t* pairs, const float* pair_coef, int32_t P,
                  const float* row_weight, const float* class_weight, const float* loss_weight4_host, float* terms, float* g_logits,
                  float* g_center, float* g_size, float* g_ortho6d, int32_t* class_scratch, parq_stream stream) {
    return parq_set_loss_flags(pred_logits, center_unnormalized, size_unnormalized, ortho6d, I, B, Q, num_classes, t_center, t_size, t_rot,
                               t_label, t_sym, nmax, pairs, pair_coef, P, row_weight, class_weight, loss_weight4_host, terms, g_logits,
                               g_center, g_size, g_ortho6d, class_scratch, 0, stream);
}

size_t parq_set_loss_scratch_bytes(int32_t I, int32_t B, int32_t Q, int32_t P, int32_t flags) {
    if (I < 1 || B < 1 || Q < 1 || P < 0 || (flags & ~PARQ_SETLOSS_DETERMINISTIC)) return 0;
    const int64_t rows = (int64_t)I * B * Q;
    return (size_t)(rows + ((flags & PARQ_SETLOSS_DETERMINISTIC) ? setloss_part_floats(P, rows) : 0)) * 4;
}

int parq_set_loss_flags(const float* pred_logits, const float* center_unnormalized, const float* size_unnormalized, const float* ortho6d,
                        int32_t I, int32_t B, int32_t Q, int32_t num_classes, const float* t_center, const float* t_size, const float* t_rot,
                        const int32_t* t_label, const int32_t* t_sym, int32_t nmax, const int32_t* pairs, const float* pair_coef, int32_t P,
                        const float* row_weight, const float* class_weight, const float* loss_weight4_host, float* terms, float* g_logits,
                        float* g_center, float* g_size, float* g_ortho6d, int32_t* class_scratch, int32_t flags, parq_stream stream) {
    if (flags & ~PARQ_SETLOSS_DETERMINISTIC) return fail(PARQ_ERR_ARG, "unknown set-loss flags 0x%x", (unsigned)flags);
    if (!pred_logits || !center_unnormalized || !size_unnormalized || !ortho6d || !t_center || !t_size || !t_rot || !t_label || !row_weight ||
        !class_weight || !loss_weight4_host || !terms || !g_logits || !g_center || !g_size || !g_ortho6d || !class_scratch)
        return fail(PARQ_ERR_ARG, "NULL argument");
    if (I < 1 || B < 1 || Q < 1 || num_classes < 2 || nmax < 1 || P < 0 || (P > 0 && (!pairs || !pair_coef))) return fail(PARQ_ERR_ARG, "bad dims");
    float* det_part = (flags & PARQ_SETLOSS_DETERMINISTIC) ? reinterpret_cast<float*>(class_scratch + (int64_t)I * B * Q) : nullptr;
    HIPCHK(launch_set_loss(pred_logits, center_unnormalized, size_unnormalized, ortho6d, I, B, Q, num_classes, t_center, t_size, t_rot,
                           t_label, t_sym, nmax, pairs, pair_coef, P, row_weight, class_weight, loss_weight4_host, num_classes - 1, terms,
                           g_logits, g_center, g_size, g_ortho6d, class_scratch, (hipStream_t)stream, det_part));
    return PARQ_OK;
}

int parq_k_layernorm(const float* X, const float* gamma, const float* beta, float* Y, int32_t M, int32_t C, float eps,
                     parq_stream stream) {
    if (!X || !gamma || !beta || !Y || M < 1 || C < 1 || C > 1024) return fail(PARQ_ERR_ARG, "bad argument");
    HIPCHK(launch_layernorm(X, gamma, beta, Y, M, C, eps, (hipStream_t)stream));
    return PARQ_OK;
}

}
```

parq_amd/csrc/common.hpp:

```cpp
#pragma once

#include <hip/hip_runtime.h>
#include <stdint.h>
#include <stddef.h>
#include <stdlib.h>

namespace parq {

typedef float f32x4 __attribute__((ext_vector_type(4)));
typedef float f32x16 __attribute__((ext_vector_type(16)));

#ifdef PARQ_DEV_PROBES
inline const char* dev_env(const char* name) { return getenv(name); }
#else
inline const char* dev_env(const char*) { return nullptr; }
#endif

enum : int { kTlLinear = 1, kTlProjectSample = 2, kTlSelfAttn = 3, kTlFlashSplit = 4, kTlFlashMerge = 5, kTlBoxDecode = 6, kTlPosemb = 7,
             kTlKvProj = 8, kTlChain = 9 };
#ifdef PARQ_DEV_PROBES
static __device__ unsigned long long* parq_tl_buf = nullptr;
static __device__ unsigned int parq_tl_cap = 0;
struct TlStamp {
    unsigned long long t0, idx; int id;
// ... 27 lines not shown
        }
    }
};
#define PARQ_TL_KERNEL(id) ::parq::TlStamp parq_tl_stamp_(id)
#ifdef PARQ_TL_MARKS
#define PARQ_TL_MARK() parq_tl_stamp_.mark()
#else
#define PARQ_TL_MARK() do { } while (0)
#endif
#define PARQ_TL_DEFINE_SETTER(fn)                                                                              \
    hipError_t fn(unsigned long long* buf, unsigned int cap) {                                                 \
        hipError_t e = hipMemcpyToSymbol(HIP_SYMBOL(parq_tl_buf), &buf, sizeof(buf));                          \
        if (e != hipSuccess) return e;                                                                         \
        return hipMemcpyToSymbol(HIP_SYMBOL(parq_tl_cap), &cap, sizeof(cap));                                  \
    }
hipError_t tl_set_linear(unsigned long long*, unsigned int);
hipError_t tl_set_elementwise(unsigned long long*, unsigned int);
hipError_t tl_set_flash(unsigned long long*, unsigned int);
hipError_t tl_set_flash_split(unsigned long long*, unsigned int);
hipError_t tl_set_flash_split8(unsigned long long*, unsigned int);
hipError_t tl_set_kvproj_split(unsigned long long*, unsigned int);
hipError_t tl_set_chain(unsigned long long*, unsigned int);
#else
#define PARQ_TL_KERNEL(id) do { } while (0)
#define PARQ_TL_MARK() do { } while (0)
#define PARQ_TL_DEFINE_SETTER(fn)
#endif

constexpr int kWave = 64;
constexpr int kGnSlots = 256;

__device__ __forceinline__ void lds_dma16(const void* gsrc, unsigned lds_base) {
    const unsigned base = __builtin_amdgcn_readfirstlane(lds_base);
    unsigned saved;
    asm volatile("s_mov_b32 %0, m0\n\ts_mov_b32 m0, %1\n\ts_nop 0\n\tglobal_load_lds_dwordx4 %2, off\n\ts_mov_b32 m0, %0"
                 : "=&s"(saved)
                 : "s"(base), "v"(gsrc)
                 : "memory");
}
__device__ __forceinline__ void lds_barrier() {
    asm volatile("s_waitcnt lgkmcnt(0)" ::: "memory");
    __builtin_amdgcn_s_barrier();
    asm volatile("" ::: "memory");
}

struct DynLdsOnce {
    unsigned long long done = 0;
    hipError_t ensure(const void* fn, size_t bytes) {
        int dev = 0;
        hipError_t e = hipGetDevice(&dev);
        if (e != hipSuccess) return e;
        const bool track = dev >= 0 && dev < 64;
        if (track && ((done >> dev) & 1ull)) return hipSuccess;
        e = hipFuncSetAttribute(fn, hipFuncAttributeMaxDynamicSharedMemorySize, (int)bytes);
        if (e == hipSuccess && track) done |= 1ull << dev;
        return e;
    }
};

__host__ __device__ inline int ceil_div(int a, int b) { return (a + b - 1) / b; }
__host__ __device__ inline int64_t ceil_div64(int64_t a, int64_t b) { return (a + b - 1) / b; }

__device__ __forceinline__ int mfma32_row(int reg, int lane) {
    return (reg & 3) + 8 * (reg >> 2) + 4 * (lane >> 5);
}

typedef _Float16 half2v __attribute__((ext_vector_type(2)));
typedef _Float16 half8 __attribute__((ext_vector_type(8)));

__device__ __forceinline__ void split_pair(float x0, float x1, half2v& hi, half2v& lo) {
    const auto h = __builtin_amdgcn_cvt_pkrtz(x0, x1);
    hi = __builtin_bit_cast(half2v, h);
    float d0, d1;
    const unsigned int hp = __builtin_bit_cast(unsigned int, h);
    asm("v_fma_mix_f32 %0, %1, -1.0, %2 op_sel_hi:[1,0,0]" : "=v"(d0) : "v"(hp), "v"(x0));
    asm("v_fma_mix_f32 %0, %1, -1.0, %2 op_sel:[1,0,0] op_sel_hi:[1,0,0]" : "=v"(d1) : "v"(hp), "v"(x1));
    lo = __builtin_bit_cast(half2v, __builtin_amdgcn_cvt_pkrtz(d0, d1));
}

__device__ __forceinline__ void split8(const float* x, half8& hi, half8& lo) {
#pragma unroll
    for (int e = 0; e < 8; e += 2) {
        half2v h, l;
        split_pair(x[e], x[e + 1], h, l);
        hi[e] = h[0]; hi[e + 1] = h[1];
        lo[e] = l[0]; lo[e + 1] = l[1];
    }
}

__device__ __forceinline__ float clamp_e4m3(float x) { return __builtin_amdgcn_fmed3f(x, -448.f, 448.f); }
__device__ __forceinline__ int pack4_e4m3(float a, float b, float c, float d) {
    const int w = __builtin_amdgcn_cvt_pk_fp8_f32(clamp_e4m3(a), clamp_e4m3(b), 0, false);
    return __builtin_amdgcn_cvt_pk_fp8_f32(clamp_e4m3(c), clamp_e4m3(d), w, true);
}
__device__ __forceinline__ void split_rtz(float x0, float x1, unsigned& hi, float& d0, float& d1) {
    hi = __builtin_bit_cast(unsigned, __builtin_amdgcn_cvt_pkrtz(x0, x1));
    asm("v_fma_mix_f32 %0, %1, -1.0, %2 op_sel_hi:[1,0,0]" : "=v"(d0) : "v"(hi), "v"(x0));
    asm("v_fma_mix_f32 %0, %1, -1.0, %2 op_sel:[1,0,0] op_sel_hi:[1,0,0]" : "=v"(d1) : "v"(hi), "v"(x1));
}
constexpr float kLo8Scale = 1024.f;
typedef int i32x4 __attribute__((ext_vector_type(4)));
__device__ __forceinline__ void pieces_e4m3(const float* x, i32x4& hi8, i32x4& lo8) {
#pragma unroll
    for (int w = 0; w < 4; ++w) {
        unsigned h0, h1;
        float d[4];
        split_rtz(x[4 * w], x[4 * w + 1], h0, d[0], d[1]);
        split_rtz(x[4 * w + 2], x[4 * w + 3], h1, d[2], d[3]);
        hi8[w] = pack4_e4m3(x[4 * w], x[4 * w + 1], x[4 * w + 2], x[4 * w + 3]);
        lo8[w] = pack4_e4m3(d[0] * kLo8Scale, d[1] * kLo8Scale, d[2] * kLo8Scale, d[3] * kLo8Scale);
    }
}
constexpr int kStage8Bytes = 24576;
constexpr int kS8Kh16 = 0, kS8K8hi = 8192, kS8K8lo = 12288, kS8Vh16 = 16384;

__host__ __device__ constexpr uint32_t rng_mix(uint32_t x) {
    x ^= x >> 16; x *= 0x7feb352dU; x ^= x >> 15; x *= 0x846ca68bU; x ^= x >> 16;
    return x;
}
__host__ __device__ inline uint32_t rng_stream(uint32_t base, uint32_t stream) { return rng_mix(base ^ rng_mix(stream * 0x9e3779b9U + 0x85ebca6bU)); }
__host__ __device__ inline uint32_t drop_rowhash(uint32_t seed, uint32_t row) { return rng_mix(seed ^ (row * 0x9e3779b1U)); }
__host__ __device__ constexpr uint32_t drop_blockhash(uint32_t blk) { return rng_mix(blk * 0x85ebca77U + 0x6a09e667U); }
__host__ __device__ constexpr uint32_t drop_regpart(uint32_t r) { return rng_mix(0x3c6ef372U + r); }
constexpr uint32_t kDropBit2Part = rng_mix(0xa54ff53aU);
__host__ __device__ constexpr uint32_t drop_colhash(uint32_t col) {
    const uint32_t k = col & 31u;
    return drop_blockhash(col >> 5) ^ drop_regpart((k & 3u) | ((k >> 3) << 2)) ^ ((k & 4u) ? kDropBit2Part : 0u);
}
__host__ __device__ inline uint32_t drop_threshold(float p) {
    const float t = ceilf(p * 16777216.0f);
    return t >= 16777216.0f ? 0xffffffffU : ((uint32_t)t << 8);
}
__host__ __device__ inline bool drop_keep_h(uint32_t rowhash, uint32_t colhash, uint32_t thr) {
    uint32_t h = ((rowhash ^ colhash) & 0xffffffU) * 0x9E3779U;
    h ^= h >> 16;
    h = (h & 0xffffffU) * 0x85EBCBU;
    return h >= thr;
}
__host__ __device__ inline bool drop_keep(uint32_t rowhash, uint32_t col, float p) {
    return drop_keep_h(rowhash, drop_colhash(col), drop_threshold(p));
}

enum : int { kF16 = 0, kBF16 = 1 };
typedef __bf16 bf16x8 __attribute__((ext_vector_type(8)));

template <int KIND>
__device__ __forceinline__ half8 cvt8_rn(const float* x) {
    if constexpr (KIND == kF16) {
        half8 h;
#pragma unroll
        for (int e = 0; e < 8; ++e) h[e] = (_Float16)x[e];
        return h;
    } else {
        bf16x8 h;
#pragma unroll
        for (int e = 0; e < 8; ++e) h[e] = (__bf16)x[e];
        return __builtin_bit_cast(half8, h);
    }
}

enum : int { kTokF32 = 0, kTokF16 = 1, kTokBF16 = 2 };
template <int TT> struct TokElem { typedef float type; };
template <> struct TokElem<kTokF16> { typedef _Float16 type; };
template <> struct TokElem<kTokBF16> { typedef unsigned short type; };
template <int TT> constexpr int tok_bytes() { return TT == kTokF32 ? 4 : 2; }

__device__ __forceinline__ float bf16_bits_to_f32(unsigned int b) { return __builtin_bit_cast(float, b << 16); }

typedef unsigned int u32x4 __attribute__((ext_vector_type(4)));
template <int TT>
__device__ __forceinline__ unsigned int round2_tok16(float y0, float y1) {
    static_assert(TT != kTokF32, "16-bit token types only");
    if constexpr (TT == kTokF16) {
        unsigned int r;
        asm("v_cvt_pk_f16_f32 %0, %1, %2" : "=v"(r) : "v"(y0), "v"(y1));
        return r;
    } else {
        typedef __bf16 bf16x2 __attribute__((ext_vector_type(2)));
        const bf16x2 v = {(__bf16)y0, (__bf16)y1};
        return __builtin_bit_cast(unsigned int, v);
    }
}
template <int TT>
__device__ __forceinline__ void widen8(u32x4 raw, float* x) {
    static_assert(TT != kTokF32, "16-bit token types only");
    const unsigned int w[4] = {raw[0], raw[1], raw[2], raw[3]};
#pragma unroll
    for (int i = 0; i < 4; ++i) {
        if constexpr (TT == kTokF16) {
            const half2v h = __builtin_bit_cast(half2v, w[i]);
            x[2 * i] = (float)h[0];
            x[2 * i + 1] = (float)h[1];
        } else {
            x[2 * i] = bf16_bits_to_f32(w[i] & 0xffffu);
            x[2 * i + 1] = bf16_bits_to_f32(w[i] >> 16);
        }
    }
}

template <int TT>
__device__ __forceinline__ f32x4 load_tok4(const void* row, int c4) {
    if constexpr (TT == kTokF32) {
        return reinterpret_cast<const f32x4*>(row)[c4];
    } else {
        const uint2 r = reinterpret_cast<const uint2*>(row)[c4];
        if constexpr (TT == kTokF16) {
            const half2v a = __builtin_bit_cast(half2v, r.x), b = __builtin_bit_cast(half2v, r.y);
            return f32x4{(float)a[0], (float)a[1], (float)b[0], (float)b[1]};
        } else {
            return f32x4{bf16_bits_to_f32(r.x & 0xffffu), bf16_bits_to_f32(r.x >> 16), bf16_bits_to_f32(r.y & 0xffffu),
                         bf16_bits_to_f32(r.y >> 16)};
        }
    }
}

template <int KIND>
__device__ __forceinline__ f32x16 mfma16(half8 a, half8 b, f32x16 c) {
    if constexpr (KIND == kF16) return __builtin_amdgcn_mfma_f32_32x32x16_f16(a, b, c, 0, 0, 0);
    else return __builtin_amdgcn_mfma_f32_32x32x16_bf16(__builtin_bit_cast(bf16x8, a), __builtin_bit_cast(bf16x8, b), c, 0, 0, 0);
}

struct LinearArgs {
    const float* X;  int64_t ldx;
    const float* X2; int64_t ldx2;
    int x2_ncols;
    const float* W;  int64_t ldw;
    const float* bias;
    const float* R;  int64_t ldr;
    float* Y;
    int M, N, K;
    int relu;
    const float* relu_mask; int64_t ldmask;
    float mask_scale;
    float drop_p; uint32_t drop_seed;
    int rows_per_batch; int64_t y_batch; int64_t y_row; int col_blk; int64_t y_blk;
    float norm_eps;
    const float* ln_gamma; const float* ln_beta; float* ln_stats_out;
    const float* rln_stats; const float* rln_gamma; const float* rln_beta;
    const double* gn_sums; const float* gn_gamma; const float* gn_beta;
    int gn_rows_per_scene; int gn_ngroups;
    double* gn_out_sums; int gn_out_ncols; int gn_out_group_cols; int gn_out_rows_per_scene; int gn_out_ngroups;
    int64_t gX, gW, gBias, gY, gGamma;
    const float* W2; const float* W2p;
    const float* Wp;
    const float* Wh; const float* wh_scale;
    const float* wh_bias; int wh_fold;
    int tile_map;
    double* lnp_out;
    unsigned* lnp_flags; unsigned lnp_epoch;
    const int* pub_flags; int* pub_mirror; int* pub_word; const int* pub_epoch; int pub_mask; int pub_peaky;
};
__device__ __forceinline__ void publish_progress(const LinearArgs& a) {
    if (a.pub_word != nullptr && blockIdx.x == 0 && blockIdx.y == 0 && threadIdx.x == 0) {
        const int f0 = a.pub_flags[0] & a.pub_mask, pk = a.pub_peaky ? a.pub_flags[1] : 0;
        const int bits = ((f0 & ~4) ? 1 : 0) | (f0 & 4) | (pk != 0 ? (2 | (pk << 8)) : 0);
        if (bits != 0 && a.pub_mirror != nullptr) __hip_atomic_fetch_or(a.pub_mirror, bits, __ATOMIC_RELAXED, __HIP_MEMORY_SCOPE_SYSTEM);
        __hip_atomic_store(a.pub_word, *a.pub_epoch, __ATOMIC_RELEASE, __HIP_MEMORY_SCOPE_SYSTEM);
    }
}
struct SeamArgs {
    const float* X1; int64_t ldx1; const float* W1p;
    const float* X2; int64_t ldx2; const float* W2p;
    const float* X3; int64_t ldx3; const float* W3p;
    const float* ln1_stats; const float* ln1_g; const float* ln1_b;
    const float* b1; const float* srow; const float* b2;
    float* Y; int64_t ldy; int M, N;
    const double* part; const unsigned* flags; unsigned epoch; int nparts; int width;
    float eps;
    float* ln_out;
    double* gn_out_sums; int gn_out_ncols; int gn_out_group_cols; int gn_out_rows_per_scene; int gn_out_ngroups;
    int* err;
};
hipError_t launch_linear(const LinearArgs& a, int groups, hipStream_t s);
hipError_t launch_chain_linear(const LinearArgs& a, int groups, hipStream_t s);
bool chain_linear_supported(const LinearArgs& a, int groups);
hipError_t launch_seam_q(const LinearArgs& xa, const SeamArgs& q, hipStream_t s);
hipError_t launch_ln_fold(const float* W, const float* b, const float* gamma, const float* beta, int R, int C, float* Wg, float* srow, float* bb, hipStream_t s);
hipError_t launch_matmul_fold(const float* A, const float* Bm, const float* bv, int R, int C, float* out, float* ob, hipStream_t s);
hipError_t launch_pack_w_half(const float* W, int64_t ldw, int N, int K, float* dst, float* scales, hipStream_t s, const float* gamma = nullptr,
                              const float* beta = nullptr, const float* bias = nullptr, float* bias_out = nullptr);
hipError_t launch_pack_w_tiles(const float* W, int64_t ldw, int N, int K, float* dst, hipStream_t s);
hipError_t launch_fold_pos_weights(const float* Wa, const float* ba, const float* W2, const float* b2, int R, int C, float* out_w, float* out_b, hipStream_t s);

struct FlashArgs {
    const float* q; int64_t q_batch, q_head, q_row;
    const float* k; int64_t k_batch, k_head, k_row;
    const float* v; int64_t v_batch, v_head, v_row;
    int B, H, Lq, Lk, dh;
    int nsplit;
    float* o_part;
    float* m_part;
    float* l_part;
    float* out; int64_t out_batch, out_row;
    float defer_log2;
    float* lse;
    float drop_p; uint32_t drop_seed;
    int flags;
    int* peaky; float peaky_l;
    int* peaky_it; int* peaky_min;
    int* head_min;
    int nh; unsigned long long hmap;
    int64_t cache_head_bytes;
};
struct FlashHead { int b, h, bh; };
__device__ __forceinline__ FlashHead flash_head(const FlashArgs& a, int z) {
    FlashHead r;
    if (a.nh > 0) { r.b = z / a.nh; r.h = (int)((a.hmap >> (4 * (z - r.b * a.nh))) & 15ull); }
    else { r.b = z / a.H; r.h = z - r.b * a.H; }
    r.bh = r.b * a.H + r.h;
    return r;
}
inline int flash_launch_heads(const FlashArgs& a) { return a.nh > 0 ? a.nh : a.H; }
int flash_key_tile(int dh);
int flash_lq_pad(int Lq);
int flash_pick_nw(int B, int H, int Lq, int Lk, int dh, int num_cus);
int flash_pick_splits(int B, int H, int Lq, int Lk, int dh, int num_cus);
int device_num_cus();
size_t flash_scratch_bytes(int B, int H, int Lq, int dh, int nsplit);
hipError_t launch_flash(const FlashArgs& a, hipStream_t s);
hipError_t launch_flash_merge(const FlashArgs& a, hipStream_t s);

size_t kvsplit_cache_bytes(int B, int H, int N, int terms = 3);
int flash_split_pick_splits(int B, int H, int Lq, int Lk, int num_cus);
size_t kvproj_big_scratch_floats(int B, int N, int C);
hipError_t launch_kvproj_big(const void* tokens, const void* Whi, const void* Wlo, const float* bias, int B, int N, int C,
                             void* cache, int* overflow, float* scratch, hipStream_t s, int terms = 3, int kind = kF16,
                             int tok_type = kTokF32);
int flash_split256_pick_splits(int B, int H, int Lq, int Lk, int num_cus);
hipError_t launch_flash_split256(const FlashArgs& a, const void* cache, hipStream_t s, int terms = 3, int kind = kF16);
hipError_t launch_kvsplit_convert(const float* K, const float* V, int64_t k_batch, int64_t k_head, int64_t k_row,
                                  int64_t v_batch, int64_t v_head, int64_t v_row, int B, int H, int N, void* cache,
                                  int* overflow_flag, hipStream_t s, int terms = 3, int kind = kF16);
hipError_t launch_kvsplit_to_f32(const void* cache, int B, int H, int N, float* K, float* V, int64_t k_batch, int64_t k_head,
                                 int64_t v_batch, int64_t v_head, hipStream_t s, int chunks = 1,
                                 int terms = 3, int kind = kF16);
hipError_t launch_flash_split(const FlashArgs& a, const void* cache, hipStream_t s, int terms = 3,
                              int kind = kF16);
bool flash_split8_supported(int dh, int Lk);
hipError_t launch_kvsplit8_convert(const float* K, const float* V, int64_t k_batch, int64_t k_head, int64_t k_row, int64_t v_batch,
                                   int64_t v_head, int64_t v_row, int B, int H, int N, void* cache, hipStream_t s);
hipError_t launch_flash_split8(const FlashArgs& a, const void* cache, hipStream_t s);
hipError_t launch_flash_single_stage(const FlashArgs& a, const void* cache, hipStream_t s, int kind);
hipError_t launch_split_f32(const float* src, void* hi, void* lo, int64_t n, hipStream_t s);
constexpr int kGatherMax = 64;
struct GatherArgs { const float* src[kGatherMax]; float* dst[kGatherMax]; int64_t n[kGatherMax]; int count; };
hipError_t launch_gather_copy(const GatherArgs& g, hipStream_t s);
hipError_t launch_set_loss(const float* logits, const float* center, const float* size, const float* o6, int I, int B, int Q, int ncls,
                           const float* t_center, const float* t_size, const float* t_rot, const int32_t* t_label, const int32_t* t_sym,
                           int nmax, const int32_t* pairs, const float* coef, int P, const float* row_weight, const float* class_weight,
                           const float* w4, int background, float* terms, float* g_logits, float* g_center, float* g_size, float* g_o6,
                           int32_t* cls, hipStream_t s, float* det_part = nullptr);
inline int64_t setloss_part_floats(int64_t P, int64_t rows) { return 3 * ((P + 255) / 256) + (rows + 255) / 256; }
hipError_t launch_kvproj_split(const void* tokens, const void* Whi, const void* Wlo, const float* bias, int B, int N,
                               int C, int H, void* cache, int* overflow, hipStream_t s, int terms = 3, int kind = kF16, unsigned safe_mask = 0,
                               int tok_type = kTokF32);
hipError_t launch_cvt16(const float* src, void* dst, int64_t n, int kind, hipStream_t s);
hipError_t launch_widen_tokens(const void* src, float* dst, int64_t n, int tok_type, hipStream_t s);
hipError_t launch_cvt16_tokens(const void* src, void* dst, int64_t n, int kind, int tok_type, hipStream_t s);

struct FpnDev {
    const float* lv[4];
    int h[4], w[4];
    int layer, cl;
};
hipError_t launch_raype_points(const float* cam, const float* T_cp, const float* T_wp, const float* T_wl,
                               const float* scale6, float min_depth, float max_depth, int B, int V, int h, int w, int S,
                               float* P, hipStream_t s);
hipError_t launch_raype_fused(const float* cam, const float* T_cp, const float* T_wp, const float* T_wl, const float* scale6,
                              float min_depth, float max_depth, int B, int V, int h, int w, const void* W1hi, const void* W1lo,
                              const float* b1, const void* W2hi, const void* W2lo, const float* b2, const float* feat,
                              float* hidden, double* Tl, double* depth, float* out, int nchw_out, hipStream_t s,
                              void* W2f = nullptr, int two_kernels = 0,
                              int out16 = kTokF32,
                              const FpnDev* fpn = nullptr);
hipError_t launch_fpn_backward(const float* d_tokens, int BV, const FpnDev& fpn, float* const* d_level, hipStream_t s);
__device__ __forceinline__ void gn_mean_rstd(double S, double Q, double inv_cnt, float eps, float& mean, float& rstd) {
    const double mu = S * inv_cnt;
    double var = Q * inv_cnt - mu * mu;
    var = var < 0.0 ? 0.0 : var;
    mean = (float)mu;
    rstd = (float)(1.0 / sqrt(var + (double)eps));
}
struct ScaleBox { float lo[3]; float hi[3]; };
struct DetScratch {
    float* base = nullptr;
    int64_t floats = 0;
};
const DetScratch* det_scratch();
struct DetScope {
    DetScratch saved;
    DetScope(float* base, int64_t floats);
    ~DetScope();
};
int64_t det_scratch_floats(int64_t sample_rows, int64_t dq_floats);
int64_t det_attn_dq_floats(int B, int H, int Lq, int Lk);
int64_t det_kvbwd_floats();
hipError_t launch_slab_reduce(const float* part, int S, int64_t stride, int R, int cols, float* out, int64_t ldo, int accumulate,
                              hipStream_t s);
hipError_t launch_gn_moments_det(const float* x, int64_t ldx, int C, int ngroups, int rows_per_scene, int B, double* sums, hipStream_t s);
hipError_t launch_transpose(const float* src, int64_t ld_src, float* dst, int64_t ld_dst, int R, int Cc, hipStream_t s);
hipError_t launch_gemm_tn(const float* A, int64_t lda, const float* B, int64_t ldb, float* out, int64_t ldo, int M, int N, int K,
                          int accumulate, hipStream_t s, float* bias = nullptr, int bias_from = 0);
hipError_t launch_colsum(const float* X, int64_t ldx, int M, int N, float* out, int accumulate, hipStream_t s);
hipError_t launch_add(const float* a, const float* b, float* y, int64_t n, hipStream_t s);
hipError_t launch_axpy_rows(const float* x, int64_t ldx, float* y, int64_t ldy, int M, int N, int accumulate, hipStream_t s);
hipError_t launch_ln_bwd(const float* gy, const float* x, const float* stats, const float* gamma, float* gx, int M, int C,
                         int accumulate, float* dgamma, float* dbeta, hipStream_t s);
hipError_t launch_gn_apply(const float* x, int64_t ldx, const double* sums, const float* gamma, const float* beta, int M, int C,
                           int ngroups, int rows_per_scene, float eps, float* y, int64_t ldy, hipStream_t s);
hipError_t launch_gn_bwd(const float* x, int64_t ldx, const double* sums, const float* gamma, const float* beta, int M, int C,
                         int ngroups, int rows_per_scene, float eps, const float* gy, int64_t ldgy, float* gz, double* bsums,
                         float* gx, int64_t ldgx, float* dgamma, float* dbeta, hipStream_t s);
hipError_t launch_decode_bwd(const float* g_logits, const float* g_center, const float* g_size, const float* g_rot,
                             const float* center, const float* size, const float* ref, ScaleBox sb, int M, int ncls, int NH1, int C,
                             float* g_h3, float* g_h1, float* g_ref, hipStream_t s);
hipError_t launch_head3_bwd(const float* g_h3, const float* w3, float* g_act, int M, int C, hipStream_t s);
hipError_t launch_posemb_bwd(const float* g_emb, const float* ref, const float* dim_t, int M, float* g_ref, hipStream_t s);
hipError_t launch_refpoint_bwd(const float* g_ref, const float* ref0, int B, int Q, float* g_w, hipStream_t s);
hipError_t launch_sample_bwd(const float* tokens, const double* T_cl, const float* cam, const float* ref, ScaleBox sb, int B, int V,
                             int h, int w, int C, int Q, const float* g_tgt, float* g_tokens, float* g_ref, hipStream_t s);
hipError_t launch_attn_bwd(const float* q, int64_t q_batch, int64_t q_head, int64_t q_row, const float* k, int64_t k_batch,
                           int64_t k_head, int64_t k_row, const float* v, int64_t v_batch, int64_t v_head, int64_t v_row,
                           const float* dO, int64_t do_batch, int64_t do_head, int64_t do_row, const float* lse, const float* D,
                           float* gq, int64_t gq_batch, int64_t gq_head, int64_t gq_row, float* gk, int64_t gk_batch,
                           int64_t gk_head, int64_t gk_row, float* gv, int64_t gv_batch, int64_t gv_head, int64_t gv_row, int B, int H,
                           int Lq, int Lk, int dh, int accumulate_kv, hipStream_t s, float* gq_part = nullptr, float drop_p = 0.f,
                           uint32_t drop_seed = 0, unsigned int* absmax = nullptr,
                           float* mat_scratch = nullptr);
size_t attn_bwd_mat_scratch_floats(int Lq, int Lk, int dh);
hipError_t launch_attn_bwd_batched(const float* q, const int64_t* q_off, int64_t q_batch, int64_t q_head, int64_t q_row, const float* k,
                                   int64_t k_batch, int64_t k_head, int64_t k_row, const float* v, int64_t v_batch, int64_t v_head,
                                   int64_t v_row, const float* dO, int64_t do_it, int64_t do_batch, int64_t do_head, int64_t do_row,
                                   const float* lse, const int64_t* lse_off, const float* D, int64_t D_it, float* gq, int64_t gq_it,
                                   int64_t gq_batch, int64_t gq_head, int64_t gq_row, float* gk, int64_t gk_batch, int64_t gk_head,
                                   int64_t gk_row, float* gv, int64_t gv_batch, int64_t gv_head, int64_t gv_row, int B, int H, int Lq,
                                   int Lk, int dh, int n_it, hipStream_t s, float* gq_part, float drop_p, const uint32_t* seeds,
                                   unsigned int* absmax, unsigned int* kv_absmax = nullptr,
                                   void* pack = nullptr,
                                   float* mat_scratch = nullptr,
                                   const void* kvcache = nullptr, int cache_terms = 0, int cache_kind = 0);
size_t attn_bwd_pack_floats(int B, int H, int Lq, int n_it);
bool kvproj_bwd_split_supported(int C);
hipError_t launch_tn_split_512x256(const float* g, int64_t ldg, const float* x, int64_t ldx, int64_t M, float* out, int64_t ldo,
                                   float* db, const unsigned int* absmax_bits, float* scale_scratch, hipStream_t s);
hipError_t launch_kvproj_bwd_split(const float* g, const float* tokens, int64_t M, int C, float* dW, float* db,
                                   const unsigned int* absmax_bits, float* scale_scratch, hipStream_t s);
hipError_t launch_dropout_apply(const float* src, float* dst, int M, int N, float p, uint32_t seed, hipStream_t s);
size_t attn_bwd_dq_partial_floats(int B, int H, int Lq, int Lk, int dh, bool grouped = false);
int attn_bwd_kb_group(int B, int H, int Lk);
size_t attn_bwd_batched256_scratch_floats(int n_it, int Lq, int Lk);
hipError_t launch_absmax(const float* x, int64_t n, unsigned int* out, hipStream_t s);
hipError_t launch_attn_bwd_rowdot(const float* dO, const float* O, int64_t batch, int64_t row, int B, int H, int Lq, int dh, float* D,
                                  hipStream_t s);
hipError_t launch_parse_pred(const float* center, const float* size, const float* rot6, const float* prob, int B, int Q, int ncls,
                             int num_semcls, const float* track_scale6, int for_vis, int enable_nms, float* obbs,
                             unsigned char* mask, hipStream_t s);
hipError_t launch_obb_iou(const double* boxes_a, const double* boxes_b, const int64_t* seg, int S, int64_t total, int64_t n_a_total,
                          int64_t n_b_total, double* iou3, double* iou2, hipStream_t s);
hipError_t launch_gemm_split(const float* X, int64_t ldx, const void* Whi, const void* Wlo, const float* bias, float* Y,
                             int64_t ldy, int M, int N, int K, int relu, const float* feat, int hw, hipStream_t s,
                             const float* scale_dev = nullptr, float scale_mul = 1.f, const float* xscale_dev = nullptr,
                             int accumulate = 0,
                             int out16 = kTokF32,
                             const FpnDev* fpn = nullptr);

hipError_t launch_camera_local(const float* T_cp, const float* T_wp, const float* T_wl, int B, int V,
                               float* T_cl, hipStream_t s);
hipError_t launch_camera_local_f64(const float* T_cp, const float* T_wp, const float* T_wl, int B, int V,
                                   double* T_cl, hipStream_t s);
hipError_t launch_initial_ref(const float* refpoint_w, int B, int Q, float* ref, hipStream_t s);
struct CallPtrs { const void* p[8]; };
struct PrologueCall { const float* cam_src; float* cam_dst; int ncam; const void** ind; CallPtrs ptrs; };
hipError_t launch_forward_prologue(const float* T_cp, const float* T_wp, const float* T_wl, int B, int V, double* T_cl, const float* w, int Q,
                                   float* ref, const float* dim_t, float* emb, float* flags, int nflags, hipStream_t s,
                                   const PrologueCall* call = nullptr);
hipError_t launch_posemb(const float* ref, const float* dim_t, int M, float* emb, hipStream_t s);
hipError_t launch_zero_f64(double* p, int n, hipStream_t s);
hipError_t launch_project_sample(const float* tokens, const float* T_cl, const float* cam, const float* ref,
                                 ScaleBox sb, int B, int V, int h, int w, int C, int Q, float* tgt,
                                 float* coord_pos, hipStream_t s);
hipError_t launch_project_sample_f64(const void* tokens, const double* T_cl, const float* cam, const float* ref,
                                     ScaleBox sb, int B, int V, int h, int w, int C, int Q, float* tgt,
                                     float* coord_pos, double* zero_f64, int zero_n, hipStream_t s, float* raw_count = nullptr,
                                     const void* const* ind = nullptr, int64_t coord_off = 0, int tok_type = kTokF32);
hipError_t launch_pe1_sample(const LinearArgs& pe1, const void* tokens, const double* T_cl, const float* cam, const float* ref, ScaleBox sb,
                             int B, int V, int h, int w, int C, int Q, float* tgt, float* coord_pos, double* zero_f64, int zero_n,
                             float* raw_count, hipStream_t s, const void* const* ind = nullptr, int64_t coord_off = 0, int tok_type = kTokF32);
hipError_t launch_sample_finalize(const float* sums, const float* counts, int64_t M, int C, float* tgt, hipStream_t s,
                                  const float* range_sum = nullptr, int* range_flag = nullptr);
hipError_t launch_shard_range_flag(const int* range_flag, float* out, hipStream_t s);
hipError_t launch_attn_combine(const float* parts, int R, int64_t rec, int B, int H, int Q, int Lq_pad, int dh, float* out, hipStream_t s);
hipError_t launch_self_attn(const float* qkv, int64_t row_stride, int B, int H, int Lq, int dh, float* out,
                            int64_t out_row, hipStream_t s, float* lse = nullptr, float drop_p = 0.f, uint32_t drop_seed = 0);
hipError_t launch_layernorm(const float* X, const float* gamma, const float* beta, float* Y, int M, int C,
                            float eps, hipStream_t s);
hipError_t launch_gn_stats(const float* X, int64_t ldx, int col0, int ncols, int ngroups, int B,
                           int rows_per_scene, float eps, float* stats, hipStream_t s);
struct BoxDecodeArgs {
    const float* h1; int64_t ld1;
    const float* h2; int64_t ld2;
    const double* gn_sums;
    const float* gn_gamma; const float* gn_beta;
    const float* w3; const float* b3;
    int C; int rows_per_scene; float eps;
    const float* ref;
    const float* mean_sizes; int n_mean;
    const float* dim_t;
    ScaleBox sb; int M; int ncls;
    float *logits, *center, *size, *rot, *prob;
    float* ref_next;
    float* emb_next;
    int* poison_mirror;
    const int* peaky;
    int peaky_poison;
    const int* poison;
    int poison_mask;
    const void* const* ind;
    int64_t out_row0;
};
hipError_t launch_box_decode(const BoxDecodeArgs& a, hipStream_t s);
hipError_t launch_copy_rows(const float* src, int64_t src_ld, float* dst, int64_t dst_ld, int rows, int cols,
                            hipStream_t s);
hipError_t launch_fill(float* dst, float value, int64_t n, hipStream_t s);

}
```

parq_amd/csrc/flash_split8.hip:

```cpp
#include "common.hpp"
#include <cstdlib>
#include <type_traits>

namespace parq {

namespace {

typedef int i32x8 __attribute__((ext_vector_type(8)));
typedef unsigned int u32x4 __attribute__((ext_vector_type(4)));

constexpr int kDH = 64, kNW = 8, kRing = 4;
constexpr int kStageBytes = kStage8Bytes;
constexpr int oKh16 = kS8Kh16, oK8hi = kS8K8hi, oK8lo = kS8K8lo, oVh16 = kS8Vh16;
constexpr float kDefer8 = 2.f;
constexpr int kE8One = 127, kE8Lo = 117;

__device__ __forceinline__ int dmap(int kh, int s, int e) { return 32 * (s >> 1) + 16 * (s & 1) + 4 * kh + (e & 3) + 8 * (e >> 2); }

__global__ __launch_bounds__(256) void kvsplit8_convert_kernel(const float* __restrict__ K, const float* __restrict__ V, int64_t k_batch,
                                                               int64_t k_head, int64_t k_row, int64_t v_batch, int64_t v_head,
                                                               int64_t v_row, int H, int N, unsigned char* __restrict__ cache) {
    __shared__ float ks[64][65];
    __shared__ float vs[64][65];
    const int st = blockIdx.x, bh = blockIdx.y, tid = threadIdx.x;
    const int b = bh / H, h = bh - b * H;
    const int nst = N / 64;
    const float* kp = K + (int64_t)b * k_batch + (int64_t)h * k_head;
    const float* vp = V + (int64_t)b * v_batch + (int64_t)h * v_head;
    for (int i = tid; i < 64 * 64; i += 256) {
        const int key = i >> 6, d = i & 63;
        const int64_t n = (int64_t)st * 64 + key;
        ks[key][d] = kp[n * k_row + d];
        vs[key][d] = vp[n * v_row + d];
    }
    __syncthreads();
    unsigned char* out = cache + ((int64_t)bh * nst + st) * kStageBytes;
#pragma unroll
    for (int b2 = 0; b2 < 2; ++b2) {
        {
            const int key = tid >> 3, c = tid & 7, kh = c >> 2, s = c & 3;
            float x[8];
#pragma unroll
            for (int e = 0; e < 8; ++e) x[e] = ks[32 * b2 + key][dmap(kh, s, e)];
            const int pos = c ^ ((key >> 1) & 7);
            half8 hi, lo;
            split8(x, hi, lo);
            *reinterpret_cast<half8*>(out + oKh16 + b2 * 4096 + (key * 64 + pos * 8) * 2) = hi;
        }
        {
            const int d = tid >> 2, c = tid & 3, m = c >> 1, kh = c & 1;
            float x[8];
#pragma unroll
            for (int e = 0; e < 8; ++e) x[e] = vs[32 * b2 + 16 * m + 4 * kh + (e & 3) + 8 * (e >> 2)][d];
            const int pos = c ^ ((d >> 2) & 3);
            *reinterpret_cast<half8*>(out + oVh16 + b2 * 4096 + (d * 32 + pos * 8) * 2) = cvt8_rn<kF16>(x);
        }
    }
    {
        const int b2 = tid >> 7, c = (tid >> 6) & 1, hh = (tid >> 5) & 1, key = tid & 31;
        float x[16];
#pragma unroll
        for (int m = 0; m < 2; ++m)
#pragma unroll
            for (int e = 0; e < 8; ++e) x[8 * m + e] = ks[32 * b2 + key][32 * m + 16 * c + 4 * hh + (e & 3) + 8 * (e >> 2)];
        i32x4 hi8, lo8;
        pieces_e4m3(x, hi8, lo8);
        *reinterpret_cast<i32x4*>(out + oK8hi + tid * 16) = hi8;
        *reinterpret_cast<i32x4*>(out + oK8lo + tid * 16) = lo8;
    }
}

__device__ __forceinline__ void xhalf_swap(float v, float& lo_bcast, float& hi_bcast) {
    float a = v, b = v;
    asm volatile("s_nop 1\n\tv_permlane32_swap_b32 %0, %1" : "+v"(a), "+v"(b));
    lo_bcast = a;
    hi_bcast = b;
}
__device__ __forceinline__ float xhalf_max(float v) {
    float a, b, o;
    xhalf_swap(v, a, b);
    asm("v_max_f32 %0, %1, %2" : "=v"(o) : "v"(a), "v"(b));
    return o;
}
__device__ __forceinline__ float xhalf_sum(float v) {
    float a, b;
    xhalf_swap(v, a, b);
    return a + b;
}

__device__ __forceinline__ f32x16 mx64(i32x8 a, i32x8 b, f32x16 c, int scale_a, int scale_b) {
    return __builtin_amdgcn_mfma_scale_f32_32x32x64_f8f6f4(a, b, c, 0, 0, 0, scale_a, 0, scale_b);
}

template <int PROBE = 0, int RING = kRing, bool REV = false, bool DROP = false, int TERMS = 8, int KIND = kF16>
__global__ __launch_bounds__(kNW * 64) void flash_split8_kernel(FlashArgs a, const unsigned char* __restrict__ cache) {
    PARQ_TL_KERNEL(kTlFlashSplit);
    static_assert(TERMS == 8 || TERMS == 1, "mode 4 or a single 16-bit product");
    static_assert(TERMS == 1 || KIND == kF16, "the split is an fp16 split");
    extern __shared__ __attribute__((aligned(16))) unsigned char smem[];
    constexpr bool MX = TERMS == 8;
    constexpr int kStageBytes = MX ? kStage8Bytes : 16384;
    auto k16_off = [](int pb) { return MX ? oKh16 + pb * 4096 : pb * 8192; };
    auto v16_off = [](int pb) { return MX ? oVh16 + pb * 4096 : pb * 8192 + 4096; };
    constexpr int NT = kNW * 64;
    constexpr int STAGE16 = kStageBytes / 16;
    constexpr int LD = STAGE16 / NT;
    static_assert(STAGE16 % NT == 0, "whole DMA rows per stage");
    constexpr int AHEAD = RING - 3;

    const int split = blockIdx.x;
    const FlashHead fh = flash_head(a, blockIdx.z);
    const int bh = fh.bh, b = fh.b, h = fh.h;
    const int tid = threadIdx.x, lane = tid & 63, wave = __builtin_amdgcn_readfirstlane(tid >> 6);
    const int li = lane & 31, kh = lane >> 5;
    const int q0 = (blockIdx.y * kNW + wave) * 32;
    const int q = q0 + li;
    const bool active = q0 < a.Lq;
    const int Lq_pad = (a.Lq + 31) & ~31;

    half8 qh[4];
    i32x8 q8h, q8l;
    {
        const float scale = 1.4426950408889634f / sqrtf((float)kDH);
        const float* qp = a.q + (int64_t)b * a.q_batch + (int64_t)h * a.q_head + (int64_t)(q < a.Lq ? q : 0) * a.q_row;
#pragma unroll
        for (int s = 0; s < 4; ++s) {
            const int d0 = 32 * (s >> 1) + 16 * (s & 1) + 4 * kh;
            f32x4 x0 = *reinterpret_cast<const f32x4*>(qp + d0);
            f32x4 x1 = *reinterpret_cast<const f32x4*>(qp + d0 + 8);
            if (q >= a.Lq) { x0 = f32x4{0.f, 0.f, 0.f, 0.f}; x1 = x0; }
            float x[8], dl[8];
            unsigned hw[4];
#pragma unroll
            for (int e = 0; e < 8; ++e) x[e] = (e < 4 ? x0[e & 3] : x1[e & 3]) * scale;
            if constexpr (!MX) { qh[s] = cvt8_rn<KIND>(x); continue; }
#pragma unroll
            for (int e = 0; e < 8; e += 2) split_rtz(x[e], x[e + 1], hw[e >> 1], dl[e], dl[e + 1]);
            qh[s] = __builtin_bit_cast(half8, u32x4{hw[0], hw[1], hw[2], hw[3]});
            const int m = s >> 1, c = s & 1;
            q8h[4 * c + 2 * m] = pack4_e4m3(x[0], x[1], x[2], x[3]);
            q8h[4 * c + 2 * m + 1] = pack4_e4m3(x[4], x[5], x[6], x[7]);
            q8l[4 * c + 2 * m] = pack4_e4m3(dl[0] * kLo8Scale, dl[1] * kLo8Scale, dl[2] * kLo8Scale, dl[3] * kLo8Scale);
            q8l[4 * c + 2 * m + 1] = pack4_e4m3(dl[4] * kLo8Scale, dl[5] * kLo8Scale, dl[6] * kLo8Scale, dl[7] * kLo8Scale);
        }
    }

    const int nst = a.Lk / 64;
    const int t_begin = (int)((int64_t)split * nst / a.nsplit);
    const int t_end = (int)((int64_t)(split + 1) * nst / a.nsplit);
    const uint4* gsrc = reinterpret_cast<const uint4*>(cache + (int64_t)bh * (a.cache_head_bytes ? a.cache_head_bytes : (int64_t)nst * kStageBytes));
    const int nbk = 2 * (t_end - t_begin);

    typedef __attribute__((address_space(3))) unsigned char lds_byte;
    auto gload = [&](int st, int slot) {
#pragma unroll
        for (int i = 0; i < LD; ++i) {
            const int64_t idx = (int64_t)st * STAGE16 + tid + i * NT;
            lds_byte* dst = (lds_byte*)(smem) + ((size_t)slot * STAGE16 + i * NT + wave * 64) * 16;
            __builtin_amdgcn_global_load_lds(gsrc + idx, dst, 16, 0, 0);
        }
    };
    constexpr bool rev = REV;
    auto src_stage = [&](int j) { return rev ? t_end - 1 - j : t_begin + j; };
    auto stage_of = [&](int n) -> const unsigned char* { return smem + (size_t)((n >> 1) % RING) * kStageBytes; };
    auto pblk = [&](int n) { return rev ? 1 - (n & 1) : (n & 1); };

#pragma unroll
    for (int j = 0; j < RING - 1; ++j)
        if (t_begin + j < t_end) gload(src_stage(j), j);
    asm volatile("s_waitcnt vmcnt(0)" ::: "memory");
    __syncthreads();
    auto sync_point = [&](int j) {
        if constexpr (!(PROBE & 8)) {
            if (AHEAD >= 2 && t_begin + j + 3 < t_end) asm volatile("s_waitcnt vmcnt(%0)" ::"n"(LD) : "memory");
            else asm volatile("s_waitcnt vmcnt(0)" ::: "memory");
            __builtin_amdgcn_s_barrier();
        }
        if (t_begin + j + RING - 1 < t_end) gload(src_stage(j + RING - 1), (j + RING - 1) % RING);
    };

    f32x16 o[2], sacc[2];
    half8 Ph[2][2];
#pragma unroll
    for (int d = 0; d < 2; ++d)
#pragma unroll
        for (int r = 0; r < 16; ++r) o[d][r] = 0.f;
#pragma unroll
    for (int c = 0; c < 2; ++c)
#pragma unroll
        for (int m = 0; m < 2; ++m) Ph[c][m] = half8{0, 0, 0, 0, 0, 0, 0, 0};
    float m_run = 0.f, l_run = 0.f, l_a = 0.f, l_b = 0.f;
    f32x16 negm16 = {0.f, 0.f, 0.f, 0.f, 0.f, 0.f, 0.f, 0.f, 0.f, 0.f, 0.f, 0.f, 0.f, 0.f, 0.f, 0.f};
    half8 kf[4], vh[2];
    i32x8 k8h, k8l;
    if constexpr (PROBE & 16) { kf[0] = qh[0]; kf[1] = qh[1]; kf[2] = qh[2]; kf[3] = qh[3]; k8h = q8h; k8l = q8l; vh[0] = qh[0]; vh[1] = qh[1]; }
    const int ksw = (li >> 1) & 7;

    auto load_k16 = [&](int n) {
        if constexpr (PROBE & 16) return;
        const _Float16* Kb = reinterpret_cast<const _Float16*>(stage_of(n) + k16_off(pblk(n)));
#pragma unroll
        for (int s = 0; s < 4; ++s) {
            const int pos = (4 * kh + s) ^ ksw;
            kf[s] = *reinterpret_cast<const half8*>(Kb + li * 64 + pos * 8);
        }
    };
    auto load_k8 = [&](int n) {
        if constexpr ((PROBE & 16) || !MX) return;
        const unsigned char* st = stage_of(n);
        const int pb = pblk(n);
#pragma unroll
        for (int c = 0; c < 2; ++c) {
            const int off = (((pb * 2 + c) * 2 + kh) * 32 + li) * 16;
            const i32x4 hv = *reinterpret_cast<const i32x4*>(st + oK8hi + off);
            const i32x4 lv = *reinterpret_cast<const i32x4*>(st + oK8lo + off);
#pragma unroll
            for (int w = 0; w < 4; ++w) { k8h[4 * c + w] = hv[w]; k8l[4 * c + w] = lv[w]; }
        }
    };
    auto load_v = [&](int n, int m, half8 (&vh)[2]) {
        if constexpr (PROBE & 16) { vh[0] = qh[0]; vh[1] = qh[1]; return; }
        const _Float16* Vb = reinterpret_cast<const _Float16*>(stage_of(n) + v16_off(pblk(n)));
#pragma unroll
        for (int dt = 0; dt < 2; ++dt) {
            const int d = dt * 32 + li;
            const int pos = (2 * m + kh) ^ ((d >> 2) & 3);
            vh[dt] = *reinterpret_cast<const half8*>(Vb + d * 32 + pos * 8);
        }
    };
    auto block_max = [&](const f32x16& S) -> float {
        float m0 = fmaxf(S[0], S[1]), m1 = fmaxf(S[8], S[9]);
#pragma unroll
        for (int r = 2; r < 8; ++r) { m0 = fmaxf(m0, S[r]); m1 = fmaxf(m1, S[8 + r]); }
        return xhalf_max(fmaxf(m0, m1));
    };
    const uint32_t drop_rh = DROP ? drop_rowhash(a.drop_seed, (uint32_t)(bh * a.Lq + q)) : 0u;
    const uint32_t drop_thr = DROP ? drop_threshold(a.drop_p) : 0u;
    const uint32_t drop_rkh = drop_rh ^ (kh ? kDropBit2Part : 0u);
    uint32_t dbase = 0u;
    auto load_drop = [&](int n) {
        if constexpr (DROP) dbase = drop_rkh ^ drop_blockhash((uint32_t)(rev ? 2 * t_end - 1 - n : 2 * t_begin + n));
    };
    typedef float f32x2p __attribute__((ext_vector_type(2)));
    typedef __bf16 bf16x2p __attribute__((ext_vector_type(2)));
    auto pack_sum = [&](float p0, float p1, float& l) -> unsigned {
        if constexpr (KIND == kF16) {
            const half2v hp = __builtin_convertvector(f32x2p{p0, p1}, half2v);
            l = __builtin_amdgcn_fdot2(hp, half2v{(_Float16)1.f, (_Float16)1.f}, l, false);
            return __builtin_bit_cast(unsigned, hp);
        } else {
            const bf16x2p bp = __builtin_convertvector(f32x2p{p0, p1}, bf16x2p);
            l = __builtin_amdgcn_fdot2_f32_bf16(bp, bf16x2p{(__bf16)1.f, (__bf16)1.f}, l, false);
            return __builtin_bit_cast(unsigned, bp);
        }
    };
    auto sm_pair = [&](auto cur, auto jj) {
        if constexpr (PROBE & 1) return;
        constexpr int CUR = decltype(cur)::value, J = decltype(jj)::value, M = J >> 2, W = J & 3;
        const float p0 = __builtin_amdgcn_exp2f(sacc[CUR][2 * J]);
        const float p1 = __builtin_amdgcn_exp2f(sacc[CUR][2 * J + 1]);
        unsigned hw;
        if constexpr ((J & 1) == 0) hw = pack_sum(p0, p1, l_a);
        else hw = pack_sum(p0, p1, l_b);
        if constexpr (DROP)
            hw &= (drop_keep_h(dbase, drop_regpart(2 * J), drop_thr) ? 0xffffu : 0u) | (drop_keep_h(dbase, drop_regpart(2 * J + 1), drop_thr) ? 0xffff0000u : 0u);
        u32x4 h4 = __builtin_bit_cast(u32x4, Ph[CUR][M]);
        h4[W] = hw;
        Ph[CUR][M] = __builtin_bit_cast(half8, h4);
    };
#define PARQ_FENCE() do { if constexpr ((PROBE & 32) != 0) __builtin_amdgcn_sched_barrier(0); } while (0)
    auto step = [&](auto cur, int n) {
        constexpr int CUR = decltype(cur)::value, NXT = CUR ^ 1;
        using IC = std::integral_constant<int, CUR>;
        const int nk = n + 2 < nbk ? n + 2 : nbk - 1;
        load_drop(n);
#define PARQ_Q(i, Bq) if constexpr (!(PROBE & 4)) sacc[NXT] = mfma16<KIND>(kf[i], Bq, (i) == 0 ? negm16 : sacc[NXT]); PARQ_FENCE()
#define PARQ_P(D, Bp) if constexpr (!(PROBE & 2)) o[D] = mfma16<KIND>(vh[D], Bp, o[D]); PARQ_FENCE()
#define PARQ_S(J) sm_pair(IC{}, std::integral_constant<int, J>{}); PARQ_FENCE()
        PARQ_Q(0, qh[0]);
        PARQ_P(0, Ph[NXT][0]);  PARQ_S(0);
        PARQ_Q(1, qh[1]);
        PARQ_P(1, Ph[NXT][0]);  PARQ_S(1);
        load_v(n > 0 ? n - 1 : 0, 1, vh);
        PARQ_FENCE();
        PARQ_Q(2, qh[2]);  PARQ_S(2);
        PARQ_Q(3, qh[3]);
        load_k16(nk);
        PARQ_FENCE();
        PARQ_S(3);
        if constexpr (!(PROBE & 4) && MX) sacc[NXT] = mx64(k8l, q8h, sacc[NXT], kE8Lo, kE8One);
        PARQ_FENCE();
        PARQ_S(4);
        PARQ_P(0, Ph[NXT][1]);  PARQ_S(5);
        if constexpr (!(PROBE & 4) && MX) sacc[NXT] = mx64(k8h, q8l, sacc[NXT], kE8One, kE8Lo);
        PARQ_FENCE();
        load_k8(nk);
        PARQ_FENCE();
        PARQ_S(6);
        PARQ_P(1, Ph[NXT][1]);  PARQ_S(7);
        load_v(n, 0, vh);
        PARQ_FENCE();
#undef PARQ_Q
#undef PARQ_P
#undef PARQ_S
        float mx_lane;
        {
            const f32x16& S = sacc[NXT];
            float m0 = fmaxf(S[0], S[1]), m1 = fmaxf(S[8], S[9]);
#pragma unroll
            for (int r = 2; r < 8; ++r) { m0 = fmaxf(m0, S[r]); m1 = fmaxf(m1, S[8 + r]); }
            mx_lane = fmaxf(m0, m1);
        }
        if (__any(mx_lane > a.defer_log2)) {
            const float mx = xhalf_max(mx_lane);
            const float d = mx > a.defer_log2 ? ceilf(mx) : 0.f;
            const float alpha = __builtin_ldexpf(1.f, -(int)d);
            m_run += d;
            l_run *= alpha;
            l_a *= alpha;
            l_b *= alpha;
#pragma unroll
            for (int dd = 0; dd < 2; ++dd)
#pragma unroll
                for (int r = 0; r < 16; ++r) o[dd][r] *= alpha;
#pragma unroll
            for (int r = 0; r < 16; ++r) { sacc[NXT][r] -= d; negm16[r] = -m_run; }
            if constexpr (KIND == kF16) {
                const _Float16 ah = (_Float16)alpha;
#pragma unroll
                for (int m = 0; m < 2; ++m)
#pragma unroll
                    for (int e = 0; e < 8; ++e) Ph[CUR][m][e] *= ah;
            } else {
#pragma unroll
                for (int m = 0; m < 2; ++m) {
                    bf16x8 bv = __builtin_bit_cast(bf16x8, Ph[CUR][m]);
#pragma unroll
                    for (int e = 0; e < 8; ++e) bv[e] = (__bf16)((float)bv[e] * alpha);
                    Ph[CUR][m] = __builtin_bit_cast(half8, bv);
                }
            }
        }
    };

    if ((a.flags & 1) && __builtin_amdgcn_readfirstlane(threadIdx.x) >= 256) __builtin_amdgcn_s_setprio(1);
    if (nbk > 0) {
        if (active) {
            load_k16(0);
            load_k8(0);
            const f32x16 zero16 = {0.f, 0.f, 0.f, 0.f, 0.f, 0.f, 0.f, 0.f, 0.f, 0.f, 0.f, 0.f, 0.f, 0.f, 0.f, 0.f};
#pragma unroll
            for (int s = 0; s < 4; ++s) sacc[0] = mfma16<KIND>(kf[s], qh[s], s == 0 ? zero16 : sacc[0]);
            if constexpr (MX) {
                sacc[0] = mx64(k8l, q8h, sacc[0], kE8Lo, kE8One);
                sacc[0] = mx64(k8h, q8l, sacc[0], kE8One, kE8Lo);
            }
            m_run = block_max(sacc[0]);
#pragma unroll
            for (int r = 0; r < 16; ++r) { sacc[0][r] -= m_run; negm16[r] = -m_run; }
            load_k16(1);
            load_k8(1);
            load_v(0, 0, vh);
        }
        int n = 0;
        for (; n + 2 < nbk; n += 2) {
            if (active) {
                step(std::integral_constant<int, 0>{}, n);
                step(std::integral_constant<int, 1>{}, n + 1);
            }
            sync_point(n >> 1);
        }
        if (active) {
            step(std::integral_constant<int, 0>{}, n);
            ++n;
            load_drop(n);
#pragma unroll
            for (int m = 0; m < 2; ++m) {
                unsigned hw[4];
#pragma unroll
                for (int e = 0; e < 8; e += 2) {
                    const float p0 = __builtin_amdgcn_exp2f(sacc[1][8 * m + e]), p1 = __builtin_amdgcn_exp2f(sacc[1][8 * m + e + 1]);
                    hw[e >> 1] = pack_sum(p0, p1, l_run);
                    if constexpr (DROP)
                        hw[e >> 1] &= (drop_keep_h(dbase, drop_regpart(8 * m + e), drop_thr) ? 0xffffu : 0u) |
                                      (drop_keep_h(dbase, drop_regpart(8 * m + e + 1), drop_thr) ? 0xffff0000u : 0u);
                }
                Ph[1][m] = __builtin_bit_cast(half8, u32x4{hw[0], hw[1], hw[2], hw[3]});
            }
#pragma unroll
            for (int blk = 0; blk < 2; ++blk)
#pragma unroll
                for (int m = 0; m < 2; ++m) {
                    half8 v2[2];
                    load_v(n - 1 + blk, m, v2);
#pragma unroll
                    for (int dt = 0; dt < 2; ++dt) o[dt] = mfma16<KIND>(v2[dt], Ph[blk][m], o[dt]);
                }
        }
    } else if (active) {
        m_run = -INFINITY;
    }

    if (active) {
        const int64_t pbase = (int64_t)blockIdx.z * a.nsplit + split;
        float* op = a.o_part + pbase * kDH * Lq_pad;
        if constexpr (DROP) {
            const float drop_scale = 1.f / (1.f - a.drop_p);
#pragma unroll
            for (int d = 0; d < 2; ++d)
#pragma unroll
                for (int r = 0; r < 16; ++r) o[d][r] *= drop_scale;
        }
        if (a.flags & 8) {
            __syncthreads();
            float* tr = reinterpret_cast<float*>(smem) + wave * (64 * 36);
#pragma unroll
            for (int d = 0; d < 2; ++d)
#pragma unroll
                for (int r = 0; r < 16; ++r) tr[(d * 32 + mfma32_row(r, lane)) * 36 + (lane & 31)] = o[d][r];
            asm volatile("s_waitcnt lgkmcnt(0)" ::: "memory");
            __builtin_amdgcn_wave_barrier();
            const int q0w = q - (lane & 31);
            typedef unsigned u32x4s __attribute__((ext_vector_type(4)));
            __amdgpu_buffer_rsrc_t rs = __builtin_amdgcn_make_buffer_rsrc((void*)op, 0, 0x7fffffff, 0x00020000);
#pragma unroll
            for (int i = 0; i < 8; ++i) {
                const int idx = i * 64 + lane, dim = idx >> 3, q4 = idx & 7;
                const f32x4 v = *reinterpret_cast<const f32x4*>(tr + dim * 36 + q4 * 4);
                __builtin_amdgcn_raw_buffer_store_b128(__builtin_bit_cast(u32x4s, v), rs, (int)((dim * Lq_pad + q0w + q4 * 4) * 4), 0, 16);
            }
        } else {
#pragma unroll
            for (int d = 0; d < 2; ++d)
#pragma unroll
                for (int r = 0; r < 16; ++r) op[(int64_t)(d * 32 + mfma32_row(r, lane)) * Lq_pad + q] = o[d][r];
        }
        const float l_tot = xhalf_sum(l_run + l_a + l_b);
        if (kh == 0) {
            a.m_part[pbase * Lq_pad + q] = m_run;
            a.l_part[pbase * Lq_pad + q] = l_tot;
        }
    }
}

}

bool flash_split8_supported(int dh, int Lk) { return dh == kDH && Lk >= 64 && Lk % 64 == 0; }

hipError_t launch_kvsplit8_convert(const float* K, const float* V, int64_t k_batch, int64_t k_head, int64_t k_row, int64_t v_batch,
                                   int64_t v_head, int64_t v_row, int B, int H, int N, void* cache, hipStream_t s) {
    if (!flash_split8_supported(kDH, N)) return hipErrorInvalidValue;
    hipLaunchKernelGGL(kvsplit8_convert_kernel, dim3(N / 64, B * H), dim3(256), 0, s, K, V, k_batch, k_head, k_row, v_batch, v_head,
                       v_row, H, N, reinterpret_cast<unsigned char*>(cache));
    return hipGetLastError();
}

hipError_t launch_flash_split8(const FlashArgs& a, const void* cache, hipStream_t s) {
    if (!flash_split8_supported(a.dh, a.Lk) || a.nsplit < 1 || a.nsplit > 256) return hipErrorInvalidValue;
    FlashArgs b = a;
    b.defer_log2 = kDefer8;
    static const int wt = [] { const char* e = dev_env("PARQ_FLASH_WT"); return e ? atoi(e) : 1; }();
    b.flags = ((a.flags & 2) ? 2 : 0) | ((wt && a.Lq % 256 == 0) ? 8 : 0);
    const dim3 grid(b.nsplit, ceil_div(b.Lq, 32 * kNW), b.B * flash_launch_heads(b));
    const unsigned char* c8 = reinterpret_cast<const unsigned char*>(cache);
#define PARQ_F8_LAUNCH_RR(PROBE, RING, REV)                                                                                    \
    {                                                                                                                          \
        static DynLdsOnce once;                                                                                                \
        const size_t lds = (size_t)(RING) * kStageBytes;                                                                       \
        if (hipError_t e = once.ensure(reinterpret_cast<const void*>(&flash_split8_kernel<PROBE, RING, REV>), lds); e != hipSuccess) return e; \
        hipLaunchKernelGGL((flash_split8_kernel<PROBE, RING, REV>), grid, dim3(kNW * 64), lds, s, b, c8);                       \
        return hipGetLastError();                                                                                              \
    }
#define PARQ_F8_LAUNCH(PROBE)                                                                                                  \
    {                                                                                                                          \
        if (b.flags & 2) PARQ_F8_LAUNCH_RR(PROBE, kRing, true)                                                                 \
        PARQ_F8_LAUNCH_RR(PROBE, kRing, false)                                                                                 \
    }
#define PARQ_F8_LAUNCH_DROP(REV)                                                                                               \
    {                                                                                                                          \
        static DynLdsOnce once;                                                                                                \
        const size_t lds = (size_t)kRing * kStageBytes;                                                                        \
        if (hipError_t e = once.ensure(reinterpret_cast<const void*>(&flash_split8_kernel<0, kRing, REV, true>), lds); e != hipSuccess) return e; \
        hipLaunchKernelGGL((flash_split8_kernel<0, kRing, REV, true>), grid, dim3(kNW * 64), lds, s, b, c8);                    \
        return hipGetLastError();                                                                                              \
    }
    if (b.drop_p > 0.f) { if (b.flags & 2) PARQ_F8_LAUNCH_DROP(true) PARQ_F8_LAUNCH_DROP(false) }
#ifdef PARQ_DEV_PROBES
    static const int probe = [] { const char* e = dev_env("PARQ_FLASH_PROBE"); return e ? atoi(e) : 0; }();
    switch (probe) {
        case 0: break;
        case 2: PARQ_F8_LAUNCH(2)
        case 4: PARQ_F8_LAUNCH(4)
        case 6: PARQ_F8_LAUNCH(6)
        case 8: PARQ_F8_LAUNCH(8)
        case 16: PARQ_F8_LAUNCH(16)
        case 22: PARQ_F8_LAUNCH(22)
        case 32: PARQ_F8_LAUNCH(32)
        default: return hipErrorInvalidValue;
    }
#endif
    PARQ_F8_LAUNCH(0)
#undef PARQ_F8_LAUNCH
#undef PARQ_F8_LAUNCH_RR
#undef PARQ_F8_LAUNCH_DROP
}

hipError_t launch_flash_single_stage(const FlashArgs& a, const void* cache, hipStream_t s, int kind) {
    if (!flash_split8_supported(a.dh, a.Lk) || a.nsplit < 1 || a.nsplit > 256 || (kind != kF16 && kind != kBF16)) return hipErrorInvalidValue;
    FlashArgs b = a;
    b.defer_log2 = kDefer8;
    b.flags = ((a.flags & 2) ? 2 : 0) | ((a.Lq % 256 == 0) ? 8 : 0);
    b.peaky = nullptr;
    const dim3 grid(b.nsplit, ceil_div(b.Lq, 32 * kNW), b.B * flash_launch_heads(b));
    const unsigned char* c8 = reinterpret_cast<const unsigned char*>(cache);
    constexpr int kRing1 = 6;
#define PARQ_F1_LAUNCH(REV, DROP, KIND)                                                                                        \
    {                                                                                                                          \
        static DynLdsOnce once;                                                                                                \
        const size_t lds = (size_t)kRing1 * 16384;                                                                             \
        if (hipError_t e = once.ensure(reinterpret_cast<const void*>(&flash_split8_kernel<0, kRing1, REV, DROP, 1, KIND>), lds); e != hipSuccess) return e; \
        hipLaunchKernelGGL((flash_split8_kernel<0, kRing1, REV, DROP, 1, KIND>), grid, dim3(kNW * 64), lds, s, b, c8);          \
        return hipGetLastError();                                                                                              \
    }
    const bool rev = (b.flags & 2) != 0, drop = b.drop_p > 0.f;
    if (kind == kF16) {
        if (drop) { if (rev) PARQ_F1_LAUNCH(true, true, kF16) PARQ_F1_LAUNCH(false, true, kF16) }
        if (rev) PARQ_F1_LAUNCH(true, false, kF16)
        PARQ_F1_LAUNCH(false, false, kF16)
    }
    if (drop) { if (rev) PARQ_F1_LAUNCH(true, true, kBF16) PARQ_F1_LAUNCH(false, true, kBF16) }
    if (rev) PARQ_F1_LAUNCH(true, false, kBF16)
    PARQ_F1_LAUNCH(false, false, kBF16)
#undef PARQ_F1_LAUNCH
}


PARQ_TL_DEFINE_SETTER(tl_set_flash_split8)

}
```

Baseline: 5964.

## Add two-query-tile-per-wave flash kernel form with stage options API

New measurement: 5532. -7.3%, worse.

```diff
diff --git a/__graft_entry__.py b/__graft_entry__.py
--- a/__graft_entry__.py
+++ b/__graft_entry__.py
@@ -9,6 +9,7 @@
 CSRC = os.path.join(ROOT, "parq_amd", "csrc")
 OUT = os.path.join(ROOT, "parq_amd", "_C", "libparq_hip.so")
 OUT_DEV = os.path.join(ROOT, "parq_amd", "_C", "libparq_hip_dev.so")
+FILE_FLAGS = {"flash_split8.hip": ["-mllvm", "-amdgpu-mfma-vgpr-form"]}
 
 
 def _hipcc():
@@ -30,7 +31,7 @@
     for s in srcs:
         o = os.path.join(objdir, os.path.basename(s)[:-4] + ".o")
         objs.append(o)
-        cmd = [_hipcc(), "--offload-arch=gfx950", "-O3", "-std=c++17", "-fPIC"] + list(flags) + ["-c", s, "-o", o]
+        cmd = [_hipcc(), "--offload-arch=gfx950", "-O3", "-std=c++17", "-fPIC"] + list(flags) + FILE_FLAGS.get(os.path.basename(s), []) + ["-c", s, "-o", o]
         print("[build]", " ".join(cmd))
         procs.append((cmd, subprocess.Popen(cmd)))
     for cmd, p in procs:
diff --git a/include/parq_hip.h b/include/parq_hip.h
--- a/include/parq_hip.h
+++ b/include/parq_hip.h
@@ -210,6 +210,8 @@
 int parq_k_attention_split8(const float *q, const float *k, const float *v, float *out, int32_t B, int32_t H,
                             int32_t Lq, int32_t Lk, void *scratch, size_t scratch_bytes, parq_stream stream);
 
+int parq_k_attention_stage_options(int32_t form, int32_t reverse, int32_t nh, uint64_t hmap);
+
 size_t parq_k_attention_split256_scratch_bytes(int32_t B, int32_t H, int32_t Lq, int32_t Lk);
 int parq_k_attention_split256(const float *q, const float *k, const float *v, float *out, int32_t B, int32_t H,
                               int32_t Lq, int32_t Lk, void *scratch, size_t scratch_bytes, parq_stream stream);
diff --git a/parq_amd/_lib.py b/parq_amd/_lib.py
--- a/parq_amd/_lib.py
+++ b/parq_amd/_lib.py
@@ -111,6 +111,7 @@
     "parq_k_attention_split_scratch_bytes": (_sz, [_i32, _i32, _i32, _i32]),
     "parq_k_attention_split": (C.c_int, [_vp, _vp, _vp, _vp, _i32, _i32, _i32, _i32, _vp, _sz, _vp]),
     "parq_k_attention_split8": (C.c_int, [_vp, _vp, _vp, _vp, _i32, _i32, _i32, _i32, _vp, _sz, _vp]),
+    "parq_k_attention_stage_options": (C.c_int, [_i32, _i32, _i32, C.c_uint64]),
     "parq_k_attention_split256_scratch_bytes": (_sz, [_i32, _i32, _i32, _i32]),
     "parq_k_attention_split256": (C.c_int, [_vp, _vp, _vp, _vp, _i32, _i32, _i32, _i32, _vp, _sz, _vp]),
     "parq_k_attention_half_scratch_bytes": (_sz, [_i32, _i32, _i32, _i32]),
diff --git a/parq_amd/csrc/api.hip b/parq_amd/csrc/api.hip
--- a/parq_amd/csrc/api.hip
+++ b/parq_amd/csrc/api.hip
@@ -1849,6 +1849,27 @@
     return PARQ_OK;
 }
 
+static struct { int form, reverse, nh; unsigned long long hmap; } g_stage_opt = {0, 0, 0, 0ull};
+
+int parq_k_attention_stage_options(int32_t form, int32_t reverse, int32_t nh, uint64_t hmap) {
+    if (form < 0 || form > 2) return fail(PARQ_ERR_ARG, "bad kernel form");
+    if (nh < 0 || nh > 16) return fail(PARQ_ERR_ARG, "bad head count");
+    g_stage_opt = {form, reverse != 0, nh, (unsigned long long)hmap};
+    return PARQ_OK;
+}
+
+static int apply_stage_options(FlashArgs& fa) {
+    fa.flags = (g_stage_opt.form == 1 ? kFlashOneTile : g_stage_opt.form == 2 ? kFlashTwoTile : 0) | (g_stage_opt.reverse ? 2 : 0);
+    if (g_stage_opt.nh > 0) {
+        if (g_stage_opt.nh > fa.H || fa.H > 16) return fail(PARQ_ERR_ARG, "head list longer than the head count");
+        for (int i = 0; i < g_stage_opt.nh; ++i)
+            if ((int)((g_stage_opt.hmap >> (4 * i)) & 15ull) >= fa.H) return fail(PARQ_ERR_ARG, "head list names a head past the head count");
+        fa.nh = g_stage_opt.nh;
+        fa.hmap = g_stage_opt.hmap;
+    }
+    return PARQ_OK;
+}
+
 int parq_k_attention_split8(const float* q, const float* k, const float* v, float* out, int32_t B, int32_t H, int32_t Lq,
                             int32_t Lk, void* scratch, size_t scratch_bytes, parq_stream stream) {
     if (!q || !k || !v || !out || !scratch) return fail(PARQ_ERR_ARG, "NULL argument");
@@ -1869,6 +1890,7 @@
     fa.o_part = (float*)(cache + kvsplit_cache_bytes(B, H, Lk));
     fa.m_part = fa.o_part + (int64_t)B * H * fa.nsplit * dh * lp;
     fa.l_part = fa.m_part + (int64_t)B * H * fa.nsplit * lp;
+    if (int e = apply_stage_options(fa)) return e;
     HIPCHK(launch_kvsplit8_convert(k, v, Lk * C, dh, C, Lk * C, dh, C, B, H, Lk, cache, s));
     HIPCHK(launch_flash_split8(fa, cache, s));
     HIPCHK(launch_flash_merge(fa, s));
@@ -1934,6 +1956,8 @@
     fa.m_part = fa.o_part + (int64_t)B * H * fa.nsplit * dh * lp;
     fa.l_part = fa.m_part + (int64_t)B * H * fa.nsplit * lp;
     HIPCHK(hipMemsetAsync(flag, 0, 256, s));
+    if (flash_split8_supported(dh, Lk))
+        if (int e = apply_stage_options(fa)) return e;
     HIPCHK(launch_kvsplit_convert(k, v, Lk * C, dh, C, Lk * C, dh, C, B, H, Lk, cache, flag, s, 1, kind));
     HIPCHK(launch_flash_split(fa, cache, s, 1, kind));
     HIPCHK(launch_flash_merge(fa, s));
diff --git a/parq_amd/csrc/common.hpp b/parq_amd/csrc/common.hpp
--- a/parq_amd/csrc/common.hpp
+++ b/parq_amd/csrc/common.hpp
@@ -353,6 +353,7 @@
     int nh; unsigned long long hmap;
     int64_t cache_head_bytes;
 };
+constexpr int kFlashOneTile = 16, kFlashTwoTile = 32;
 struct FlashHead { int b, h, bh; };
 __device__ __forceinline__ FlashHead flash_head(const FlashArgs& a, int z) {
     FlashHead r;
diff --git a/parq_amd/csrc/flash_split8.hip b/parq_amd/csrc/flash_split8.hip
--- a/parq_amd/csrc/flash_split8.hip
+++ b/parq_amd/csrc/flash_split8.hip
@@ -10,6 +10,18 @@
 typedef unsigned int u32x4 __attribute__((ext_vector_type(4)));
 
 constexpr int kDH = 64, kNW = 8, kRing = 4;
+#ifndef PARQ_F8_RING2
+#define PARQ_F8_RING2 6
+#endif
+constexpr int kRing2 = PARQ_F8_RING2;
+#ifndef PARQ_F8_TWO_TILE
+#define PARQ_F8_TWO_TILE 0
+#endif
+constexpr bool kTwoTileMx = (PARQ_F8_TWO_TILE & 1) != 0, kTwoTileF16 = (PARQ_F8_TWO_TILE & 2) != 0, kTwoTileBF16 = (PARQ_F8_TWO_TILE & 4) != 0;
+inline bool two_tile_form(const FlashArgs& a, bool dflt) {
+    const bool applies = !(a.drop_p > 0.f) && a.Lq % 64 == 0;
+    return applies && !(a.flags & kFlashOneTile) && (dflt || (a.flags & kFlashTwoTile));
+}
 constexpr int kStageBytes = kStage8Bytes;
 constexpr int oKh16 = kS8Kh16, oK8hi = kS8K8hi, oK8lo = kS8K8lo, oVh16 = kS8Vh16;
 constexpr float kDefer8 = 2.f;
@@ -92,11 +104,18 @@
     return __builtin_amdgcn_mfma_scale_f32_32x32x64_f8f6f4(a, b, c, 0, 0, 0, scale_a, 0, scale_b);
 }
 
-template <int PROBE = 0, int RING = kRing, bool REV = false, bool DROP = false, int TERMS = 8, int KIND = kF16>
-__global__ __launch_bounds__(kNW * 64) void flash_split8_kernel(FlashArgs a, const unsigned char* __restrict__ cache) {
+template <int N, class F>
+__device__ __forceinline__ void for_tiles(F&& f) {
+    f(std::integral_constant<int, 0>{});
+    if constexpr (N > 1) f(std::integral_constant<int, 1>{});
+}
+template <int PROBE = 0, int RING = kRing, bool REV = false, bool DROP = false, int TERMS = 8, int KIND = kF16, int QT = 1>
+__global__ __launch_bounds__(kNW / QT * 64) void flash_split8_kernel(FlashArgs a, const unsigned char* __restrict__ cache) {
     PARQ_TL_KERNEL(kTlFlashSplit);
     static_assert(TERMS == 8 || TERMS == 1, "mode 4 or a single 16-bit product");
     static_assert(TERMS == 1 || KIND == kF16, "the split is an fp16 split");
+    static_assert(QT == 1 || (QT == 2 && !DROP), "one or two query tiles per wave; training keeps the one-tile form");
+    constexpr int kNW = parq::kNW / QT;
     extern __shared__ __attribute__((aligned(16))) unsigned char smem[];
     constexpr bool MX = TERMS == 8;
     constexpr int kStageBytes = MX ? kStage8Bytes : 16384;
@@ -107,20 +126,30 @@
     constexpr int LD = STAGE16 / NT;
     static_assert(STAGE16 % NT == 0, "whole DMA rows per stage");
     constexpr int AHEAD = RING - 3;
+    constexpr int INFL = QT == 2 && AHEAD >= 2 ? AHEAD : 1;
+    static_assert(RING * kStageBytes >= 8 * 64 * 36 * 4, "the write-through epilogue transposes eight tiles through the ring");
 
     const int split = blockIdx.x;
     const FlashHead fh = flash_head(a, blockIdx.z);
     const int bh = fh.bh, b = fh.b, h = fh.h;
     const int tid = threadIdx.x, lane = tid & 63, wave = __builtin_amdgcn_readfirstlane(tid >> 6);
     const int li = lane & 31, kh = lane >> 5;
-    const int q0 = (blockIdx.y * kNW + wave) * 32;
-    const int q = q0 + li;
-    const bool active = q0 < a.Lq;
+    int qv[QT];
+    bool tile_on[QT];
+    for_tiles<QT>([&](auto t) {
+        constexpr int T = decltype(t)::value;
+        const int q0 = ((blockIdx.y * kNW + wave) * QT + T) * 32;
+        qv[T] = q0 + li;
+        tile_on[T] = q0 < a.Lq;
+    });
+    const bool active = tile_on[0];
     const int Lq_pad = (a.Lq + 31) & ~31;
 
-    half8 qh[4];
-    i32x8 q8h, q8l;
-    {
+    half8 qh[QT][4];
+    i32x8 q8h[QT], q8l[QT];
+    for_tiles<QT>([&](auto t) {
+        constexpr int T = decltype(t)::value;
+        const int q = qv[T];
         const float scale = 1.4426950408889634f / sqrtf((float)kDH);
         const float* qp = a.q + (int64_t)b * a.q_batch + (int64_t)h * a.q_head + (int64_t)(q < a.Lq ? q : 0) * a.q_row;
 #pragma unroll
@@ -133,17 +162,17 @@
             unsigned hw[4];
 #pragma unroll
             for (int e = 0; e < 8; ++e) x[e] = (e < 4 ? x0[e & 3] : x1[e & 3]) * scale;
-            if constexpr (!MX) { qh[s] = cvt8_rn<KIND>(x); continue; }
+            if constexpr (!MX) { qh[T][s] = cvt8_rn<KIND>(x); continue; }
 #pragma unroll
             for (int e = 0; e < 8; e += 2) split_rtz(x[e], x[e + 1], hw[e >> 1], dl[e], dl[e + 1]);
-            qh[s] = __builtin_bit_cast(half8, u32x4{hw[0], hw[1], hw[2], hw[3]});
+            qh[T][s] = __builtin_bit_cast(half8, u32x4{hw[0], hw[1], hw[2], hw[3]});
             const int m = s >> 1, c = s & 1;
-            q8h[4 * c + 2 * m] = pack4_e4m3(x[0], x[1], x[2], x[3]);
-            q8h[4 * c + 2 * m + 1] = pack4_e4m3(x[4], x[5], x[6], x[7]);
-            q8l[4 * c + 2 * m] = pack4_e4m3(dl[0] * kLo8Scale, dl[1] * kLo8Scale, dl[2] * kLo8Scale, dl[3] * kLo8Scale);
-            q8l[4 * c + 2 * m + 1] = pack4_e4m3(dl[4] * kLo8Scale, dl[5] * kLo8Scale, dl[6] * kLo8Scale, dl[7] * kLo8Scale);
-        }
-    }
+            q8h[T][4 * c + 2 * m] = pack4_e4m3(x[0], x[1], x[2], x[3]);
+            q8h[T][4 * c + 2 * m + 1] = pack4_e4m3(x[4], x[5], x[6], x[7]);
+            q8l[T][4 * c + 2 * m] = pack4_e4m3(dl[0] * kLo8Scale, dl[1] * kLo8Scale, dl[2] * kLo8Scale, dl[3] * kLo8Scale);
+            q8l[T][4 * c + 2 * m + 1] = pack4_e4m3(dl[4] * kLo8Scale, dl[5] * kLo8Scale, dl[6] * kLo8Scale, dl[7] * kLo8Scale);
+        }
+    });
 
     const int nst = a.Lk / 64;
     const int t_begin = (int)((int64_t)split * nst / a.nsplit);
@@ -172,28 +201,36 @@
     __syncthreads();
     auto sync_point = [&](int j) {
         if constexpr (!(PROBE & 8)) {
-            if (AHEAD >= 2 && t_begin + j + 3 < t_end) asm volatile("s_waitcnt vmcnt(%0)" ::"n"(LD) : "memory");
+            if (AHEAD >= 2 && t_begin + j + 2 + INFL < t_end) asm volatile("s_waitcnt vmcnt(%0)" ::"n"(INFL * LD) : "memory");
             else asm volatile("s_waitcnt vmcnt(0)" ::: "memory");
             __builtin_amdgcn_s_barrier();
         }
         if (t_begin + j + RING - 1 < t_end) gload(src_stage(j + RING - 1), (j + RING - 1) % RING);
     };
 
-    f32x16 o[2], sacc[2];
-    half8 Ph[2][2];
-#pragma unroll
-    for (int d = 0; d < 2; ++d)
-#pragma unroll
-        for (int r = 0; r < 16; ++r) o[d][r] = 0.f;
-#pragma unroll
-    for (int c = 0; c < 2; ++c)
-#pragma unroll
-        for (int m = 0; m < 2; ++m) Ph[c][m] = half8{0, 0, 0, 0, 0, 0, 0, 0};
-    float m_run = 0.f, l_run = 0.f, l_a = 0.f, l_b = 0.f;
-    f32x16 negm16 = {0.f, 0.f, 0.f, 0.f, 0.f, 0.f, 0.f, 0.f, 0.f, 0.f, 0.f, 0.f, 0.f, 0.f, 0.f, 0.f};
+    f32x16 o[QT][2], sacc[QT][2];
+    half8 Ph[QT][2][2];
+    float m_run[QT], l_run[QT], l_a[QT], l_b[QT];
+    std::conditional_t<QT == 1, f32x16, float> negm[QT];
+    auto splat16 = [](float x) { return f32x16{x, x, x, x, x, x, x, x, x, x, x, x, x, x, x, x}; };
+    auto set_negm = [&](auto t, float x) { if constexpr (QT == 1) negm[decltype(t)::value] = splat16(x); else negm[decltype(t)::value] = x; };
+    auto get_negm = [&](auto t) -> f32x16 { if constexpr (QT == 1) return negm[decltype(t)::value]; else return splat16(negm[decltype(t)::value]); };
+    for_tiles<QT>([&](auto t) {
+        constexpr int T = decltype(t)::value;
+#pragma unroll
+        for (int d = 0; d < 2; ++d)
+#pragma unroll
+            for (int r = 0; r < 16; ++r) o[T][d][r] = 0.f;
+#pragma unroll
+        for (int c = 0; c < 2; ++c)
+#pragma unroll
+            for (int m = 0; m < 2; ++m) Ph[T][c][m] = half8{0, 0, 0, 0, 0, 0, 0, 0};
+        m_run[T] = 0.f; l_run[T] = 0.f; l_a[T] = 0.f; l_b[T] = 0.f;
+        set_negm(t, 0.f);
+    });
     half8 kf[4], vh[2];
     i32x8 k8h, k8l;
-    if constexpr (PROBE & 16) { kf[0] = qh[0]; kf[1] = qh[1]; kf[2] = qh[2]; kf[3] = qh[3]; k8h = q8h; k8l = q8l; vh[0] = qh[0]; vh[1] = qh[1]; }
+    if constexpr (PROBE & 16) { kf[0] = qh[0][0]; kf[1] = qh[0][1]; kf[2] = qh[0][2]; kf[3] = qh[0][3]; k8h = q8h[0]; k8l = q8l[0]; vh[0] = qh[0][0]; vh[1] = qh[0][1]; }
     const int ksw = (li >> 1) & 7;
 
     auto load_k16 = [&](int n) {
@@ -219,7 +256,7 @@
         }
     };
     auto load_v = [&](int n, int m, half8 (&vh)[2]) {
-        if constexpr (PROBE & 16) { vh[0] = qh[0]; vh[1] = qh[1]; return; }
+        if constexpr (PROBE & 16) { vh[0] = qh[0][0]; vh[1] = qh[0][1]; return; }
         const _Float16* Vb = reinterpret_cast<const _Float16*>(stage_of(n) + v16_off(pblk(n)));
 #pragma unroll
         for (int dt = 0; dt < 2; ++dt) {
@@ -234,7 +271,7 @@
         for (int r = 2; r < 8; ++r) { m0 = fmaxf(m0, S[r]); m1 = fmaxf(m1, S[8 + r]); }
         return xhalf_max(fmaxf(m0, m1));
     };
-    const uint32_t drop_rh = DROP ? drop_rowhash(a.drop_seed, (uint32_t)(bh * a.Lq + q)) : 0u;
+    const uint32_t drop_rh = DROP ? drop_rowhash(a.drop_seed, (uint32_t)(bh * a.Lq + qv[0])) : 0u;
     const uint32_t drop_thr = DROP ? drop_threshold(a.drop_p) : 0u;
     const uint32_t drop_rkh = drop_rh ^ (kh ? kDropBit2Part : 0u);
     uint32_t dbase = 0u;
@@ -254,19 +291,19 @@
             return __builtin_bit_cast(unsigned, bp);
         }
     };
-    auto sm_pair = [&](auto cur, auto jj) {
+    auto sm_pair = [&](auto cur, auto jj, auto t) {
         if constexpr (PROBE & 1) return;
-        constexpr int CUR = decltype(cur)::value, J = decltype(jj)::value, M = J >> 2, W = J & 3;
-        const float p0 = __builtin_amdgcn_exp2f(sacc[CUR][2 * J]);
-        const float p1 = __builtin_amdgcn_exp2f(sacc[CUR][2 * J + 1]);
+        constexpr int CUR = decltype(cur)::value, J = decltype(jj)::value, M = J >> 2, W = J & 3, T = decltype(t)::value;
+        const float p0 = __builtin_amdgcn_exp2f(sacc[T][CUR][2 * J]);
+        const float p1 = __builtin_amdgcn_exp2f(sacc[T][CUR][2 * J + 1]);
         unsigned hw;
-        if constexpr ((J & 1) == 0) hw = pack_sum(p0, p1, l_a);
-        else hw = pack_sum(p0, p1, l_b);
+        if constexpr ((J & 1) == 0) hw = pack_sum(p0, p1, l_a[T]);
+        else hw = pack_sum(p0, p1, l_b[T]);
         if constexpr (DROP)
             hw &= (drop_keep_h(dbase, drop_regpart(2 * J), drop_thr) ? 0xffffu : 0u) | (drop_keep_h(dbase, drop_regpart(2 * J + 1), drop_thr) ? 0xffff0000u : 0u);
-        u32x4 h4 = __builtin_bit_cast(u32x4, Ph[CUR][M]);
+        u32x4 h4 = __builtin_bit_cast(u32x4, Ph[T][CUR][M]);
         h4[W] = hw;
-        Ph[CUR][M] = __builtin_bit_cast(half8, h4);
+        Ph[T][CUR][M] = __builtin_bit_cast(half8, h4);
     };
 #define PARQ_FENCE() do { if constexpr ((PROBE & 32) != 0) __builtin_amdgcn_sched_barrier(0); } while (0)
     auto step = [&](auto cur, int n) {
@@ -274,73 +311,77 @@
         using IC = std::integral_constant<int, CUR>;
         const int nk = n + 2 < nbk ? n + 2 : nbk - 1;
         load_drop(n);
-#define PARQ_Q(i, Bq) if constexpr (!(PROBE & 4)) sacc[NXT] = mfma16<KIND>(kf[i], Bq, (i) == 0 ? negm16 : sacc[NXT]); PARQ_FENCE()
-#define PARQ_P(D, Bp) if constexpr (!(PROBE & 2)) o[D] = mfma16<KIND>(vh[D], Bp, o[D]); PARQ_FENCE()
-#define PARQ_S(J) sm_pair(IC{}, std::integral_constant<int, J>{}); PARQ_FENCE()
-        PARQ_Q(0, qh[0]);
-        PARQ_P(0, Ph[NXT][0]);  PARQ_S(0);
-        PARQ_Q(1, qh[1]);
-        PARQ_P(1, Ph[NXT][0]);  PARQ_S(1);
+#define PARQ_T(...) for_tiles<QT>([&](auto t) { constexpr int T = decltype(t)::value; __VA_ARGS__; }); PARQ_FENCE()
+#define PARQ_Q(i) PARQ_T(if constexpr (!(PROBE & 4)) sacc[T][NXT] = mfma16<KIND>(kf[i], qh[T][i], (i) == 0 ? get_negm(t) : sacc[T][NXT]))
+#define PARQ_P(D, M) PARQ_T(if constexpr (!(PROBE & 2)) o[T][D] = mfma16<KIND>(vh[D], Ph[T][NXT][M], o[T][D]))
+#define PARQ_S(J) PARQ_T(sm_pair(IC{}, std::integral_constant<int, J>{}, t))
+        PARQ_Q(0);
+        PARQ_P(0, 0);  PARQ_S(0);
+        PARQ_Q(1);
+        PARQ_P(1, 0);  PARQ_S(1);
         load_v(n > 0 ? n - 1 : 0, 1, vh);
         PARQ_FENCE();
-        PARQ_Q(2, qh[2]);  PARQ_S(2);
-        PARQ_Q(3, qh[3]);
+        PARQ_Q(2);  PARQ_S(2);
+        PARQ_Q(3);
         load_k16(nk);
         PARQ_FENCE();
         PARQ_S(3);
-        if constexpr (!(PROBE & 4) && MX) sacc[NXT] = mx64(k8l, q8h, sacc[NXT], kE8Lo, kE8One);
-        PARQ_FENCE();
+        PARQ_T(if constexpr (!(PROBE & 4) && MX) sacc[T][NXT] = mx64(k8l, q8h[T], sacc[T][NXT], kE8Lo, kE8One));
         PARQ_S(4);
-        PARQ_P(0, Ph[NXT][1]);  PARQ_S(5);
-        if constexpr (!(PROBE & 4) && MX) sacc[NXT] = mx64(k8h, q8l, sacc[NXT], kE8One, kE8Lo);
-        PARQ_FENCE();
+        PARQ_P(0, 1);  PARQ_S(5);
+        PARQ_T(if constexpr (!(PROBE & 4) && MX) sacc[T][NXT] = mx64(k8h, q8l[T], sacc[T][NXT], kE8One, kE8Lo));
         load_k8(nk);
         PARQ_FENCE();
         PARQ_S(6);
-        PARQ_P(1, Ph[NXT][1]);  PARQ_S(7);
+        PARQ_P(1, 1);  PARQ_S(7);
         load_v(n, 0, vh);
         PARQ_FENCE();
 #undef PARQ_Q
 #undef PARQ_P
 #undef PARQ_S
-        float mx_lane;
-        {
-            const f32x16& S = sacc[NXT];
-            float m0 = fmaxf(S[0], S[1]), m1 = fmaxf(S[8], S[9]);
-#pragma unroll
-            for (int r = 2; r < 8; ++r) { m0 = fmaxf(m0, S[r]); m1 = fmaxf(m1, S[8 + r]); }
-            mx_lane = fmaxf(m0, m1);
-        }
-        if (__any(mx_lane > a.defer_log2)) {
-            const float mx = xhalf_max(mx_lane);
-            const float d = mx > a.defer_log2 ? ceilf(mx) : 0.f;
-            const float alpha = __builtin_ldexpf(1.f, -(int)d);
-            m_run += d;
-            l_run *= alpha;
-            l_a *= alpha;
-            l_b *= alpha;
-#pragma unroll
-            for (int dd = 0; dd < 2; ++dd)
-#pragma unroll
-                for (int r = 0; r < 16; ++r) o[dd][r] *= alpha;
-#pragma unroll
-            for (int r = 0; r < 16; ++r) { sacc[NXT][r] -= d; negm16[r] = -m_run; }
-            if constexpr (KIND == kF16) {
-                const _Float16 ah = (_Float16)alpha;
-#pragma unroll
-                for (int m = 0; m < 2; ++m)
-#pragma unroll
-                    for (int e = 0; e < 8; ++e) Ph[CUR][m][e] *= ah;
-            } else {
-#pragma unroll
-                for (int m = 0; m < 2; ++m) {
-                    bf16x8 bv = __builtin_bit_cast(bf16x8, Ph[CUR][m]);
-#pragma unroll
-                    for (int e = 0; e < 8; ++e) bv[e] = (__bf16)((float)bv[e] * alpha);
-                    Ph[CUR][m] = __builtin_bit_cast(half8, bv);
+#undef PARQ_T
+        for_tiles<QT>([&](auto t) {
+            constexpr int T = decltype(t)::value;
+            float mx_lane;
+            {
+                const f32x16& S = sacc[T][NXT];
+                float m0 = fmaxf(S[0], S[1]), m1 = fmaxf(S[8], S[9]);
+#pragma unroll
+                for (int r = 2; r < 8; ++r) { m0 = fmaxf(m0, S[r]); m1 = fmaxf(m1, S[8 + r]); }
+                mx_lane = fmaxf(m0, m1);
+            }
+            if (__any(mx_lane > a.defer_log2)) {
+                const float mx = xhalf_max(mx_lane);
+                const float d = mx > a.defer_log2 ? ceilf(mx) : 0.f;
+                const float alpha = __builtin_ldexpf(1.f, -(int)d);
+                m_run[T] += d;
+                l_run[T] *= alpha;
+                l_a[T] *= alpha;
+                l_b[T] *= alpha;
+#pragma unroll
+                for (int dd = 0; dd < 2; ++dd)
+#pragma unroll
+                    for (int r = 0; r < 16; ++r) o[T][dd][r] *= alpha;
+#pragma unroll
+                for (int r = 0; r < 16; ++r) sacc[T][NXT][r] -= d;
+                set_negm(t, -m_run[T]);
+                if constexpr (KIND == kF16) {
+                    const _Float16 ah = (_Float16)alpha;
+#pragma unroll
+                    for (int m = 0; m < 2; ++m)
+#pragma unroll
+                        for (int e = 0; e < 8; ++e) Ph[T][CUR][m][e] *= ah;
+                } else {
+#pragma unroll
+                    for (int m = 0; m < 2; ++m) {
+                        bf16x8 bv = __builtin_bit_cast(bf16x8, Ph[T][CUR][m]);
+#pragma unroll
+                        for (int e = 0; e < 8; ++e) bv[e] = (__bf16)((float)bv[e] * alpha);
+                        Ph[T][CUR][m] = __builtin_bit_cast(half8, bv);
+                    }
                 }
             }
-        }
+        });
     };
 
     if ((a.flags & 1) && __builtin_amdgcn_readfirstlane(threadIdx.x) >= 256) __builtin_amdgcn_s_setprio(1);
@@ -349,15 +390,19 @@
             load_k16(0);
             load_k8(0);
             const f32x16 zero16 = {0.f, 0.f, 0.f, 0.f, 0.f, 0.f, 0.f, 0.f, 0.f, 0.f, 0.f, 0.f, 0.f, 0.f, 0.f, 0.f};
-#pragma unroll
-            for (int s = 0; s < 4; ++s) sacc[0] = mfma16<KIND>(kf[s], qh[s], s == 0 ? zero16 : sacc[0]);
-            if constexpr (MX) {
-                sacc[0] = mx64(k8l, q8h, sacc[0], kE8Lo, kE8One);
-                sacc[0] = mx64(k8h, q8l, sacc[0], kE8One, kE8Lo);
-            }
-            m_run = block_max(sacc[0]);
-#pragma unroll
-            for (int r = 0; r < 16; ++r) { sacc[0][r] -= m_run; negm16[r] = -m_run; }
+            for_tiles<QT>([&](auto t) {
+                constexpr int T = decltype(t)::value;
+#pragma unroll
+                for (int s = 0; s < 4; ++s) sacc[T][0] = mfma16<KIND>(kf[s], qh[T][s], s == 0 ? zero16 : sacc[T][0]);
+                if constexpr (MX) {
+                    sacc[T][0] = mx64(k8l, q8h[T], sacc[T][0], kE8Lo, kE8One);
+                    sacc[T][0] = mx64(k8h, q8l[T], sacc[T][0], kE8One, kE8Lo);
+                }
+                m_run[T] = block_max(sacc[T][0]);
+#pragma unroll
+                for (int r = 0; r < 16; ++r) sacc[T][0][r] -= m_run[T];
+                set_negm(t, -m_run[T]);
+            });
             load_k16(1);
             load_k8(1);
             load_v(0, 0, vh);
@@ -374,72 +419,83 @@
             step(std::integral_constant<int, 0>{}, n);
             ++n;
             load_drop(n);
-#pragma unroll
-            for (int m = 0; m < 2; ++m) {
-                unsigned hw[4];
-#pragma unroll
-                for (int e = 0; e < 8; e += 2) {
-                    const float p0 = __builtin_amdgcn_exp2f(sacc[1][8 * m + e]), p1 = __builtin_amdgcn_exp2f(sacc[1][8 * m + e + 1]);
-                    hw[e >> 1] = pack_sum(p0, p1, l_run);
-                    if constexpr (DROP)
-                        hw[e >> 1] &= (drop_keep_h(dbase, drop_regpart(8 * m + e), drop_thr) ? 0xffffu : 0u) |
-                                      (drop_keep_h(dbase, drop_regpart(8 * m + e + 1), drop_thr) ? 0xffff0000u : 0u);
+            for_tiles<QT>([&](auto t) {
+                constexpr int T = decltype(t)::value;
+#pragma unroll
+                for (int m = 0; m < 2; ++m) {
+                    unsigned hw[4];
+#pragma unroll
+                    for (int e = 0; e < 8; e += 2) {
+                        const float p0 = __builtin_amdgcn_exp2f(sacc[T][1][8 * m + e]), p1 = __builtin_amdgcn_exp2f(sacc[T][1][8 * m + e + 1]);
+                        hw[e >> 1] = pack_sum(p0, p1, l_run[T]);
+                        if constexpr (DROP)
+                            hw[e >> 1] &= (drop_keep_h(dbase, drop_regpart(8 * m + e), drop_thr) ? 0xffffu : 0u) |
+                                          (drop_keep_h(dbase, drop_regpart(8 * m + e + 1), drop_thr) ? 0xffff0000u : 0u);
+                    }
+                    Ph[T][1][m] = __builtin_bit_cast(half8, u32x4{hw[0], hw[1], hw[2], hw[3]});
                 }
-                Ph[1][m] = __builtin_bit_cast(half8, u32x4{hw[0], hw[1], hw[2], hw[3]});
-            }
+            });
 #pragma unroll
             for (int blk = 0; blk < 2; ++blk)
 #pragma unroll
                 for (int m = 0; m < 2; ++m) {
                     half8 v2[2];
                     load_v(n - 1 + blk, m, v2);
-#pragma unroll
-                    for (int dt = 0; dt < 2; ++dt) o[dt] = mfma16<KIND>(v2[dt], Ph[blk][m], o[dt]);
+                    for_tiles<QT>([&](auto t) {
+                        constexpr int T = decltype(t)::value;
+#pragma unroll
+                        for (int dt = 0; dt < 2; ++dt) o[T][dt] = mfma16<KIND>(v2[dt], Ph[T][blk][m], o[T][dt]);
+                    });
                 }
         }
     } else if (active) {
-        m_run = -INFINITY;
+        for_tiles<QT>([&](auto t) { m_run[decltype(t)::value] = -INFINITY; });
     }
 
     if (active) {
         const int64_t pbase = (int64_t)blockIdx.z * a.nsplit + split;
         float* op = a.o_part + pbase * kDH * Lq_pad;
-        if constexpr (DROP) {
-            const float drop_scale = 1.f / (1.f - a.drop_p);
-#pragma unroll
-            for (int d = 0; d < 2; ++d)
-#pragma unroll
-                for (int r = 0; r < 16; ++r) o[d][r] *= drop_scale;
-        }
-        if (a.flags & 8) {
-            __syncthreads();
-            float* tr = reinterpret_cast<float*>(smem) + wave * (64 * 36);
-#pragma unroll
-            for (int d = 0; d < 2; ++d)
-#pragma unroll
-                for (int r = 0; r < 16; ++r) tr[(d * 32 + mfma32_row(r, lane)) * 36 + (lane & 31)] = o[d][r];
-            asm volatile("s_waitcnt lgkmcnt(0)" ::: "memory");
-            __builtin_amdgcn_wave_barrier();
-            const int q0w = q - (lane & 31);
-            typedef unsigned u32x4s __attribute__((ext_vector_type(4)));
-            __amdgpu_buffer_rsrc_t rs = __builtin_amdgcn_make_buffer_rsrc((void*)op, 0, 0x7fffffff, 0x00020000);
-#pragma unroll
-            for (int i = 0; i < 8; ++i) {
-                const int idx = i * 64 + lane, dim = idx >> 3, q4 = idx & 7;
-                const f32x4 v = *reinterpret_cast<const f32x4*>(tr + dim * 36 + q4 * 4);
-                __builtin_amdgcn_raw_buffer_store_b128(__builtin_bit_cast(u32x4s, v), rs, (int)((dim * Lq_pad + q0w + q4 * 4) * 4), 0, 16);
+        if (a.flags & 8) __syncthreads();
+        for_tiles<QT>([&](auto t) {
+            constexpr int T = decltype(t)::value;
+            if (!tile_on[T]) return;
+            const int q = qv[T];
+            if constexpr (DROP) {
+                const float drop_scale = 1.f / (1.f - a.drop_p);
+#pragma unroll
+                for (int d = 0; d < 2; ++d)
+#pragma unroll
+                    for (int r = 0; r < 16; ++r) o[T][d][r] *= drop_scale;
             }
-        } else {
-#pragma unroll
-            for (int d = 0; d < 2; ++d)
-#pragma unroll
-                for (int r = 0; r < 16; ++r) op[(int64_t)(d * 32 + mfma32_row(r, lane)) * Lq_pad + q] = o[d][r];
-        }
-        const float l_tot = xhalf_sum(l_run + l_a + l_b);
-        if (kh == 0) {
-            a.m_part[pbase * Lq_pad + q] = m_run;
-            a.l_part[pbase * Lq_pad + q] = l_tot;
-        }
+            if (a.flags & 8) {
+                float* tr = reinterpret_cast<float*>(smem) + (wave * QT + T) * (64 * 36);
+#pragma unroll
+                for (int d = 0; d < 2; ++d)
+#pragma unroll
+                    for (int r = 0; r < 16; ++r) tr[(d * 32 + mfma32_row(r, lane)) * 36 + (lane & 31)] = o[T][d][r];
+                asm volatile("s_waitcnt lgkmcnt(0)" ::: "memory");
+                __builtin_amdgcn_wave_barrier();
+                const int q0w = q - (lane & 31);
+                typedef unsigned u32x4s __attribute__((ext_vector_type(4)));
+                __amdgpu_buffer_rsrc_t rs = __builtin_amdgcn_make_buffer_rsrc((void*)op, 0, 0x7fffffff, 0x00020000);
+#pragma unroll
+                for (int i = 0; i < 8; ++i) {
+                    const int idx = i * 64 + lane, dim = idx >> 3, q4 = idx & 7;
+                    const f32x4 v = *reinterpret_cast<const f32x4*>(tr + dim * 36 + q4 * 4);
+                    __builtin_amdgcn_raw_buffer_store_b128(__builtin_bit_cast(u32x4s, v), rs, (int)((dim * Lq_pad + q0w + q4 * 4) * 4), 0, 16);
+                }
+            } else {
+#pragma unroll
+                for (int d = 0; d < 2; ++d)
+#pragma unroll
+                    for (int r = 0; r < 16; ++r) op[(int64_t)(d * 32 + mfma32_row(r, lane)) * Lq_pad + q] = o[T][d][r];
+            }
+            const float l_tot = xhalf_sum(l_run[T] + l_a[T] + l_b[T]);
+            if (kh == 0) {
+                a.m_part[pbase * Lq_pad + q] = m_run[T];
+                a.l_part[pbase * Lq_pad + q] = l_tot;
+            }
+        });
     }
 }
 
@@ -463,12 +519,13 @@
     b.flags = ((a.flags & 2) ? 2 : 0) | ((wt && a.Lq % 256 == 0) ? 8 : 0);
     const dim3 grid(b.nsplit, ceil_div(b.Lq, 32 * kNW), b.B * flash_launch_heads(b));
     const unsigned char* c8 = reinterpret_cast<const unsigned char*>(cache);
-#define PARQ_F8_LAUNCH_RR(PROBE, RING, REV)                                                                                    \
+#define PARQ_F8_LAUNCH_RR(PROBE, RING, REV) PARQ_F8_LAUNCH_QT(PROBE, RING, REV, 1)
+#define PARQ_F8_LAUNCH_QT(PROBE, RING, REV, QT)                                                                                \
     {                                                                                                                          \
         static DynLdsOnce once;                                                                                                \
         const size_t lds = (size_t)(RING) * kStageBytes;                                                                       \
-        if (hipError_t e = once.ensure(reinterpret_cast<const void*>(&flash_split8_kernel<PROBE, RING, REV>), lds); e != hipSuccess) return e; \
-        hipLaunchKernelGGL((flash_split8_kernel<PROBE, RING, REV>), grid, dim3(kNW * 64), lds, s, b, c8);                       \
+        if (hipError_t e = once.ensure(reinterpret_cast<const void*>(&flash_split8_kernel<PROBE, RING, REV, false, 8, kF16, QT>), lds); e != hipSuccess) return e; \
+        hipLaunchKernelGGL((flash_split8_kernel<PROBE, RING, REV, false, 8, kF16, QT>), grid, dim3(kNW / (QT) * 64), lds, s, b, c8); \
         return hipGetLastError();                                                                                              \
     }
 #define PARQ_F8_LAUNCH(PROBE)                                                                                                  \
@@ -499,9 +556,14 @@
         default: return hipErrorInvalidValue;
     }
 #endif
+    if (two_tile_form(a, kTwoTileMx)) {
+        if (b.flags & 2) PARQ_F8_LAUNCH_QT(0, kRing2, true, 2)
+        PARQ_F8_LAUNCH_QT(0, kRing2, false, 2)
+    }
     PARQ_F8_LAUNCH(0)
 #undef PARQ_F8_LAUNCH
 #undef PARQ_F8_LAUNCH_RR
+#undef PARQ_F8_LAUNCH_QT
 #undef PARQ_F8_LAUNCH_DROP
 }
 
@@ -514,15 +576,18 @@
     const dim3 grid(b.nsplit, ceil_div(b.Lq, 32 * kNW), b.B * flash_launch_heads(b));
     const unsigned char* c8 = reinterpret_cast<const unsigned char*>(cache);
     constexpr int kRing1 = 6;
-#define PARQ_F1_LAUNCH(REV, DROP, KIND)                                                                                        \
+#define PARQ_F1_LAUNCH(REV, DROP, KIND) PARQ_F1_LAUNCH_QT(REV, DROP, KIND, 1)
+#define PARQ_F1_LAUNCH_QT(REV, DROP, KIND, QT)                                                                                 \
     {                                                                                                                          \
         static DynLdsOnce once;                                                                                                \
         const size_t lds = (size_t)kRing1 * 16384;                                                                             \
-        if (hipError_t e = once.ensure(reinterpret_cast<const void*>(&flash_split8_kernel<0, kRing1, REV, DROP, 1, KIND>), lds); e != hipSuccess) return e; \
-        hipLaunchKernelGGL((flash_split8_kernel<0, kRing1, REV, DROP, 1, KIND>), grid, dim3(kNW * 64), lds, s, b, c8);          \
+        if (hipError_t e = once.ensure(reinterpret_cast<const void*>(&flash_split8_kernel<0, kRing1, REV, DROP, 1, KIND, QT>), lds); e != hipSuccess) return e; \
+        hipLaunchKernelGGL((flash_split8_kernel<0, kRing1, REV, DROP, 1, KIND, QT>), grid, dim3(kNW / (QT) * 64), lds, s, b, c8); \
         return hipGetLastError();                                                                                              \
     }
     const bool rev = (b.flags & 2) != 0, drop = b.drop_p > 0.f;
+    if (kind == kF16 && two_tile_form(a, kTwoTileF16)) { if (rev) PARQ_F1_LAUNCH_QT(true, false, kF16, 2) PARQ_F1_LAUNCH_QT(false, false, kF16, 2) }
+    if (kind == kBF16 && two_tile_form(a, kTwoTileBF16)) { if (rev) PARQ_F1_LAUNCH_QT(true, false, kBF16, 2) PARQ_F1_LAUNCH_QT(false, false, kBF16, 2) }
     if (kind == kF16) {
         if (drop) { if (rev) PARQ_F1_LAUNCH(true, true, kF16) PARQ_F1_LAUNCH(false, true, kF16) }
         if (rev) PARQ_F1_LAUNCH(true, false, kF16)
@@ -532,6 +597,7 @@
     if (rev) PARQ_F1_LAUNCH(true, false, kBF16)
     PARQ_F1_LAUNCH(false, false, kBF16)
 #undef PARQ_F1_LAUNCH
+#undef PARQ_F1_LAUNCH_QT
 }
 
 
```
